# kpreid/all-is-cubes

Hardware: AMD Instinct MI355X
Metric: Mrays/s (higher is better)
Workload: dtype f64

## Files before the change

all_is_cubes_amd/csrc/aic_abi.cpp:

```cpp

#include <hip/hip_runtime.h>

#include <chrono>
#include <cmath>
#include <condition_variable>
#include <mutex>
#include <thread>
#include <cstdio>
#include <cstdlib>
#include <cstring>
#include <initializer_list>
#include <string>
#include <utility>
#include <vector>

#include "../../include/aic_hip.h"
#include "aic_bloom.h"
#include "aic_ctx.h"
#include "aic_device.h"
#include "aic_encode.h"
#include "aic_launch.h"

using namespace aic;

static_assert(sizeof(aic_pixel_aux) == sizeof(DevAux), "aux record layout");

static_assert(sizeof(aic_block_desc) == 48, "aic_block_desc is 48 bytes");

namespace {

constexpr uint64_t kMaxPoolElems = 0x7ffffff0ull;
constexpr uint64_t kMaxLightTexels = 0x3ffffff0ull;

}

namespace aic {

aic_options default_options() {
    aic_options o;
    std::memset(&o, 0, sizeof(o));
    o.fog = 1;
    o.transparency = 1;
    o.threshold = 0.5f;
    o.lighting = 3;
    o.maximum_intensity = INFINITY;
    o.bloom_intensity = 0.125f;
    o.view_distance = 200.0;
    return o;
}

void dump_record(aic_ctx *c, uint32_t tag, uint32_t layer, std::initializer_list<DumpPart> parts) {
    if (!c || !c->dump) return;
    uint64_t total = 0;
    for (const DumpPart &d : parts) total += d.p ? d.n : 0;
    std::fwrite(&tag, 4, 1, c->dump);
    std::fwrite(&layer, 4, 1, c->dump);
    std::fwrite(&total, 8, 1, c->dump);
    for (const DumpPart &d : parts)
        if (d.p && d.n) std::fwrite(d.p, 1, d.n, c->dump);
    std::fflush(c->dump);
}

thread_local std::string *tl_err_sink = nullptr;
int fail(aic_ctx *c, int code, const char *what, hipError_t e) {
    if (c) {
        std::string &dst = tl_err_sink ? *tl_err_sink : c->err;
        dst = what;
        if (e != hipSuccess) {
            dst += ": ";
            dst += hipGetErrorString(e);
        }
    }
    return code;
}

int hip_fail(aic_ctx *c, const char *what, hipError_t e) {
    return fail(c, e == hipErrorOutOfMemory ? AIC_ERR_OOM : AIC_ERR_DEVICE, what, e);
}

int take_light_spare(aic_ctx *c, Layer &l, int layer, size_t n, int *index) {
    auto in_use = [&](const DevBuf<uint32_t> &b) {
        for (uint32_t i = 0; i < AIC_MAX_IN_FLIGHT; i++)
            if (c->slots[i].busy && b.p && c->slots[i].light_used[layer] == (const void *)b.p) return true;
        return false;
    };
    int pick = -1;
    for (int k = 0; k < Layer::kLightSpares && pick < 0; k++)
        if (l.light_spare[k].p && l.light_spare[k].cap >= n && !in_use(l.light_spare[k])) pick = k;
    for (int k = 0; k < Layer::kLightSpares && pick < 0; k++)
        if (!l.light_spare[k].p || (l.light_spare[k].cap < n && !in_use(l.light_spare[k]))) pick = k;
    if (pick < 0) {
        pick = 0;
        for (uint32_t i = 0; i < AIC_MAX_IN_FLIGHT; i++)
            if (c->slots[i].busy && c->slots[i].light_used[layer] == (const void *)l.light_spare[0].p) {
                const hipError_t e = hipStreamSynchronize(c->slots[i].stream);
                if (e != hipSuccess) return fail(c, AIC_ERR_DEVICE, "waiting for a frame that reads a spare light volume", e);
            }
    }
    const hipError_t e = l.light_spare[pick].ensure(n);
    if (e != hipSuccess) return fail(c, e == hipErrorOutOfMemory ? AIC_ERR_OOM : AIC_ERR_DEVICE, "alloc light (spare volume)", e);
    *index = pick;
    return AIC_OK;
}

int quiesce(aic_ctx *c) {
    { const int rc = light_job_finish(c); if (rc != AIC_OK) return rc; }
    for (uint32_t i = 0; i < AIC_MAX_IN_FLIGHT; i++)
        if (c->slots[i].busy) HIP_TRY(c, hipStreamSynchronize(c->slots[i].stream));
    return AIC_OK;
}

}

namespace {

bool valid_resolution(int r) { return r >= 1 && r <= 128 && (r & (r - 1)) == 0; }

inline uint32_t block_class(const DevBlock &b) { return (b.kind & 255u) ? 2u : ((b.kind & 0x80000000u) ? 0u : 1u); }
inline void set_class(std::vector<uint32_t> &cls, uint32_t index, uint32_t c2) {
    if (cls.size() <= index / 16u) cls.resize(index / 16u + 1u, 0u);
    cls[index / 16u] = (cls[index / 16u] & ~(3u << ((index & 15u) * 2u))) | (c2 << ((index & 15u) * 2u));
}

inline bool invisible(const float *e) { return e[3] == 0.f && e[4] == 0.f && e[5] == 0.f && e[6] == 0.f; }
inline bool selectable_float_ok(float v) {
    uint32_t bits;
    std::memcpy(&bits, &v, sizeof(bits));
    return bits == 0u || bits == 0x3f800000u;
}

int convert_block(aic_ctx *c, const aic_block_desc &d, const uint16_t *voxels, const float *palette, uint32_t vox_off,
                  uint32_t pal_off, DevBlock *out, std::vector<uint16_t> *vox_out, std::vector<DevPaletteEntry> *pal_out) {
    std::memset(out, 0, sizeof(*out));
    if (!valid_resolution(d.resolution)) return fail(c, AIC_ERR_INVALID, "block resolution must be a power of two in 1..128");
    const bool one = (d.flags & AIC_BLOCK_ONE) != 0;
    const bool voxel_flag = (d.flags & AIC_BLOCK_VOXEL_SELECTABLE) != 0;
    size_t nvox = one ? 1 : (size_t)d.vsize[0] * (size_t)d.vsize[1] * (size_t)d.vsize[2];
    for (int a = 0; a < 3 && !one; a++) {
        if (d.vsize[a] < 0 || d.vlo[a] < 0 || d.vlo[a] + d.vsize[a] > d.resolution)
            return fail(c, AIC_ERR_INVALID, "block voxel bounds exceed GridAab::for_block(resolution)");
    }
    if (d.pal_len == 0 && nvox > 0) return fail(c, AIC_ERR_INVALID, "block has voxels but an empty palette");
    if (!palette && (one || d.pal_len > 0)) return fail(c, AIC_ERR_INVALID, "block has a palette length but no palette");
    if (!voxels && !one && nvox > 0) return fail(c, AIC_ERR_INVALID, "block has a voxel volume but no voxels");
    for (uint32_t i = 0; i < (one ? 1u : d.pal_len) && palette; i++) {
        const float *e = palette + 8 * (size_t)i;
        for (int k = 0; k < 7; k++)
            if (!(e[k] >= 0.f)) return fail(c, AIC_ERR_INVALID, "palette entry has a negative or NaN component");
        if (!(e[3] <= 1.f)) return fail(c, AIC_ERR_INVALID, "palette entry has alpha above 1");
        if (voxel_flag && !selectable_float_ok(e[7])) return fail(c, AIC_ERR_INVALID, "palette entry of an AIC_BLOCK_VOXEL_SELECTABLE block: the eighth float is neither 1.0f nor 0.0f");
    }
    const bool block_selectable = !(d.flags & (AIC_BLOCK_UNSELECTABLE | AIC_BLOCK_AIR));
    auto voxel_selectable = [&](const float *e) { return voxel_flag ? e[7] == 1.f : !invisible(e); };
    if (one || d.resolution == 1) {
        const float *e = nullptr;
        static const float air[8] = {0, 0, 0, 0, 0, 0, 0, 0};
        if (one) e = palette;
        else {
            bool inb = nvox > 0 && d.vlo[0] <= 0 && d.vlo[1] <= 0 && d.vlo[2] <= 0 && d.vlo[0] + d.vsize[0] > 0 &&
                       d.vlo[1] + d.vsize[1] > 0 && d.vlo[2] + d.vsize[2] > 0;
            if (inb) {
                size_t i = ((size_t)(0 - d.vlo[0]) * d.vsize[1] + (size_t)(0 - d.vlo[1])) * d.vsize[2] + (size_t)(0 - d.vlo[2]);
                uint16_t idx = voxels[i];
                if (idx >= d.pal_len) return fail(c, AIC_ERR_INVALID, "voxel index exceeds palette");
                e = palette + 8 * (size_t)idx;
            } else e = air;
        }
        out->kind = invisible(e) ? 0x80000000u : 0u;
        for (int k = 0; k < 4; k++) out->color[k] = e[k] + 0.0f;
        for (int k = 0; k < 3; k++) out->emission[k] = e[4 + k] + 0.0f;
        out->pad[0] = block_selectable && voxel_selectable(e) ? kBlockSelectable : 0u;
        return AIC_OK;
    }
    std::vector<uint32_t> remap(d.pal_len);
    uint32_t n_inv = 0;
    for (uint32_t i = 0; i < d.pal_len; i++)
        if (invisible(palette + 8 * (size_t)i)) n_inv++;
    uint32_t next_inv = 0, next_vis = n_inv;
    size_t pal_base = pal_out->size();
    pal_out->resize(pal_base + d.pal_len);
    for (uint32_t i = 0; i < d.pal_len; i++) {
        const float *e = palette + 8 * (size_t)i;
        uint32_t dst = invisible(e) ? next_inv++ : next_vis++;
        remap[i] = dst;
        DevPaletteEntry &pe = (*pal_out)[pal_base + dst];
        for (int k = 0; k < 4; k++) pe.color[k] = e[k] + 0.0f;
        for (int k = 0; k < 3; k++) pe.emission[k] = e[4 + k] + 0.0f;
        pe.pad = voxel_selectable(e) ? 1.f : 0.f;
    }
    size_t vox_base = vox_out->size();
    vox_out->resize(vox_base + nvox);
    for (size_t i = 0; i < nvox; i++) {
        uint16_t idx = voxels[i];
        if (idx >= d.pal_len) return fail(c, AIC_ERR_INVALID, "voxel index exceeds palette");
        (*vox_out)[vox_base + i] = (uint16_t)remap[idx];
    }
    out->kind = (uint32_t)d.resolution;
    out->vlo_packed = (uint32_t)d.vlo[0] | ((uint32_t)d.vlo[1] << 8) | ((uint32_t)d.vlo[2] << 16);
    out->vsize_packed = (uint32_t)d.vsize[0] | ((uint32_t)d.vsize[1] << 8) | ((uint32_t)d.vsize[2] << 16);
    out->vox_off = vox_off;
    out->pal_off = pal_off;
    out->n_invisible = n_inv;
    out->pad[0] = block_selectable ? kBlockSelectable : 0u;
    return AIC_OK;
}

}

extern "C" {

int aic_abi_version(void) { return AIC_ABI_VERSION; }

aic_ctx *aic_create(int device_id, int *status) {
    int st_dummy;
    if (!status) status = &st_dummy;
    int n = 0;
    hipError_t e = hipGetDeviceCount(&n);
    if (e != hipSuccess || n <= 0) {
        *status = AIC_ERR_NO_DEVICE;
        return nullptr;
    }
    if (device_id < 0) {
        if (hipGetDevice(&device_id) != hipSuccess) device_id = 0;
    }
    if (device_id >= n) {
        *status = AIC_ERR_INVALID;
        return nullptr;
    }
    if (hipSetDevice(device_id) != hipSuccess) {
        *status = AIC_ERR_DEVICE;
        return nullptr;
    }
    aic_ctx *c = new aic_ctx();
    c->device = device_id;
    hipDeviceProp_t prop;
    if (hipGetDeviceProperties(&prop, device_id) == hipSuccess) c->n_cus = prop.multiProcessorCount > 0 ? (uint32_t)prop.multiProcessorCount : 256u;
    if (hipGetDeviceProperties(&prop, device_id) == hipSuccess) std::snprintf(c->devname, sizeof(c->devname), "%s (%s)", prop.name, prop.gcnArchName);
    {
        auto env_int = [](const char *name, int dflt) { const char *e = std::getenv(name); return e ? std::atoi(e) : dflt; };
        c->sw.tile = env_int("AIC_TILE", 0);
        c->sw.macro = env_int("AIC_MACRO", 0);
        c->sw.feedback = env_int("AIC_TILE_FEEDBACK", 1) != 0;
        c->sw.wait_whole_stream = env_int("AIC_WAIT_WHOLE_STREAM", 0) != 0;
        c->sw.lines_clear_keys = env_int("AIC_LINES_CLEAR_KEYS", 0) != 0;
        c->sw.tiles_per_wave = (uint32_t)std::max(0, env_int("AIC_TILES_PER_WAVE", 0));
        if (const char *p = std::getenv("AIC_WAVE_PROF")) c->sw.wave_prof = p;
    }
    if (const char *path = std::getenv("AIC_DUMP")) {
        static int n_dumps = 0;
        std::string pth = path;
        if (n_dumps > 0) pth += "." + std::to_string(n_dumps);
        n_dumps++;
        c->dump = std::fopen(pth.c_str(), "wb");
        if (c->dump) std::fwrite("AICDUMP1", 1, 8, c->dump);
    }
    bool ok = hipStreamCreateWithFlags(&c->stream, hipStreamNonBlocking) == hipSuccess;
    for (uint32_t i = 0; ok && i < 8u && i < AIC_MAX_IN_FLIGHT; i++) {
        aic_ctx::FrameSlot &fs = c->slots[i];
        if (i == 0) fs.stream = c->stream;
        else ok = hipStreamCreateWithFlags(&fs.stream, hipStreamNonBlocking) == hipSuccess;
        ok = ok && hipEventCreate(&fs.ev0) == hipSuccess && hipEventCreate(&fs.ev1) == hipSuccess && hipEventCreate(&fs.ev2) == hipSuccess && fs.sub[0].counters.ensure(1) == hipSuccess;
    }
    ok = ok && hipStreamCreateWithFlags(&c->upload_stream, hipStreamNonBlocking) == hipSuccess;
    float lut[256];
    lut[0] = 0.f;
    for (int v = 1; v < 256; v++) {
        float arg = ((float)v - 144.0f) / 10.0f;
        lut[v] = (float)std::exp2((double)arg);
    }
    ok = ok && c->lut.ensure(256) == hipSuccess && hipMemcpy(c->lut.p, lut, sizeof(lut), hipMemcpyHostToDevice) == hipSuccess;
    {
        auto enc = [](float cc) -> int {
            float v = cc <= 0.0031308f ? cc * (323.f / 25.f) : (211.f * std::pow(cc, 5.f / 12.f) - 11.f) / 200.f;
            float r = std::round(v * 255.f);
            if (!(r > 0.f)) return 0;
            return r >= 255.f ? 255 : (int)r;
        };
        float thr[256];
        thr[0] = 0.f;
        for (int k = 1; k < 256; k++) {
            uint32_t lo_b = 0u, hi_b = 0x40000000u;
            while (hi_b - lo_b > 1u) {
                const uint32_t mid = lo_b + (hi_b - lo_b) / 2u;
                float f;
                std::memcpy(&f, &mid, 4);
                if (enc(f) >= k) hi_b = mid; else lo_b = mid;
            }
            for (int back = 0; back < 8 && hi_b > 1u; back++) {
                uint32_t probe = hi_b - 1u;
                float f;
                std::memcpy(&f, &probe, 4);
                bool lower_found = false;
                for (uint32_t d = 0; d < 8u && probe > d; d++) {
                    const uint32_t q = probe - d;
                    std::memcpy(&f, &q, 4);
                    if (enc(f) >= k) { hi_b = q; lower_found = true; }
                }
                if (!lower_found) break;
            }
            std::memcpy(&thr[k], &hi_b, 4);
        }
        ok = ok && c->srgb_thr.ensure(256) == hipSuccess && hipMemcpy(c->srgb_thr.p, thr, sizeof(thr), hipMemcpyHostToDevice) == hipSuccess;
        uint32_t buckets[kSrgbBucketWords];
        ok = ok && srgb8_bucket_build(thr, buckets) && c->srgb_buckets.ensure(kSrgbBucketWords) == hipSuccess &&
             hipMemcpy(c->srgb_buckets.p, buckets, sizeof(buckets), hipMemcpyHostToDevice) == hipSuccess;
    }
    if (!ok) {
        *status = AIC_ERR_DEVICE;
        aic_destroy(c);
        return nullptr;
    }
    for (auto &l : c->layers) l.opt = default_options();
    *status = AIC_OK;
    return c;
}

void aic_destroy(aic_ctx *c) {
    if (!c) return;
    (void)hipSetDevice(c->device);
    (void)light_job_finish(c);
    if (c->ljob.worker.joinable()) {
        { std::lock_guard<std::mutex> lk(c->ljob.mu); c->ljob.quit = true; }
        c->ljob.cv.notify_all();
        c->ljob.worker.join();
    }
    if (c->stream) (void)hipStreamSynchronize(c->stream);
    for (uint32_t i = 0; i < AIC_MAX_IN_FLIGHT; i++) {
        aic_ctx::FrameSlot &fs = c->slots[i];
        if (fs.stream) (void)hipStreamSynchronize(fs.stream);
        for (auto &sb : fs.sub) sb.release();
        fs.ray_cold.release(); fs.edges.release();
        if (fs.ev0) (void)hipEventDestroy(fs.ev0);
        if (fs.ev1) (void)hipEventDestroy(fs.ev1);
        if (fs.ev2) (void)hipEventDestroy(fs.ev2);
        fs.tile_static.release(); fs.queue_static.release();
        if (i > 0 && fs.stream) (void)hipStreamDestroy(fs.stream);
    }
    for (auto &l : c->layers) l.release();
    c->lut.release(); c->srgb_thr.release(); c->srgb_buckets.release(); c->out.release(); c->aux.release(); c->staging.release(); c->ortho_views.release(); c->reproject_scratch.release(); c->pick_scratch.release(); c->stale_scratch.release(); c->stale_cubes_scratch.release(); c->present_scratch.release(); c->lines_scratch.release();
    c->text_atlas.release(); c->text_codes.release(); c->export_counts.release(); c->exposure_scratch.release(); c->cursor_scratch.release();
    if (c->dump) std::fclose(c->dump);
    if (c->upload_stream) (void)hipStreamDestroy(c->upload_stream);
    if (c->stream) (void)hipStreamDestroy(c->stream);
    delete c;
}

const char *aic_last_error(const aic_ctx *c) { return c ? c->err.c_str() : "no context"; }

int aic_device_name(const aic_ctx *c, char *buf, uint32_t buf_len) {
    if (!c || !buf || !buf_len) return AIC_ERR_INVALID;
    std::snprintf(buf, buf_len, "%s", c->devname);
    return AIC_OK;
}

int aic_upload_space(aic_ctx *c, int layer, const aic_space_desc *s) {
    if (!c || !s || !valid_layer(layer)) return fail(c, AIC_ERR_INVALID, "aic_upload_space: bad argument");
    HIP_TRY(c, hipSetDevice(c->device));
    { int qrc = quiesce(c); if (qrc != AIC_OK) return qrc; }
    for (int a = 0; a < 3; a++)
        if (s->size[a] < 0 || (int64_t)s->lo[a] + s->size[a] > 2147483647LL) return fail(c, AIC_ERR_INVALID, "space bounds out of range");
    Layer &l = c->layers[layer];
    const size_t n = (size_t)s->size[0] * (size_t)s->size[1] * (size_t)s->size[2];
    if (n && (!s->block_index || !s->light)) return fail(c, AIC_ERR_INVALID, "space has cubes but no block_index/light");
    if (s->n_blocks > 65536) return fail(c, AIC_ERR_INVALID, "more than 65536 blocks");
    if (n + s->n_voxels > kMaxPoolElems) return fail(c, AIC_ERR_INVALID, "space too large (cube grid + voxel pool must stay within 4 GiB)");
    if (n > kMaxLightTexels) return fail(c, AIC_ERR_INVALID, "space too large (the light volume, 4 bytes per cube, must stay within 4 GiB)");
    if (s->n_blocks && !s->blocks) return fail(c, AIC_ERR_INVALID, "blocks is null");
    for (int o = 0; o < 8; o++)
        for (int k = 0; k < 3; k++)
            if (!(s->sky[o][k] >= 0.f)) return fail(c, AIC_ERR_INVALID, "sky colour has a negative or NaN component");

    std::vector<DevBlock> blocks(s->n_blocks);
    std::vector<uint32_t> vox_cap(s->n_blocks, 0u), pal_cap(s->n_blocks, 0u), vox_base(s->n_blocks, 0u), pal_base(s->n_blocks, 0u);
    std::vector<uint16_t> vox;
    std::vector<DevPaletteEntry> pal;
    vox.reserve((size_t)s->n_voxels);
    pal.reserve((size_t)s->n_palette);
    int32_t air_index = -1;
    for (uint32_t i = 0; i < s->n_blocks; i++) {
        const aic_block_desc &d = s->blocks[i];
        const bool one = (d.flags & AIC_BLOCK_ONE) != 0;
        size_t nvox = one ? 1 : (size_t)(d.vsize[0] > 0 ? d.vsize[0] : 0) * (size_t)(d.vsize[1] > 0 ? d.vsize[1] : 0) * (size_t)(d.vsize[2] > 0 ? d.vsize[2] : 0);
        if ((uint64_t)d.vox_off + nvox > s->n_voxels || (uint64_t)d.pal_off + d.pal_len > s->n_palette)
            return fail(c, AIC_ERR_INVALID, "block voxel/palette range exceeds the pools");
        if (n + vox.size() + nvox > kMaxPoolElems || pal.size() + d.pal_len > 0xfffffff0ull) return fail(c, AIC_ERR_INVALID, "pool too large");
        const size_t vb = vox.size(), pb = pal.size();
        int rc = convert_block(c, d, s->voxels ? s->voxels + d.vox_off : nullptr, s->palette ? s->palette + 8 * (size_t)d.pal_off : nullptr,
                               (uint32_t)(n + vox.size()), (uint32_t)pal.size(), &blocks[i], &vox, &pal);
        if (rc != AIC_OK) return rc;
        vox_cap[i] = (uint32_t)(vox.size() - vb);
        pal_cap[i] = (uint32_t)(pal.size() - pb);
        vox_base[i] = (uint32_t)(n + vb);
        pal_base[i] = (uint32_t)pb;
        if ((d.flags & AIC_BLOCK_AIR) && air_index < 0) air_index = (int32_t)i;
    }
    for (size_t i = 0; i < n; i++)
        if (s->block_index[i] >= s->n_blocks) return fail(c, AIC_ERR_INVALID, "cube block index out of range");

    hipError_t e;
    std::vector<uint32_t> cls;
    for (uint32_t i = 0; i < s->n_blocks; i++) set_class(cls, i, block_class(blocks[i]));
    if (cls.empty()) cls.push_back(0u);
    if ((e = l.pool.ensure(n + vox.size())) != hipSuccess) return hip_fail(c, "alloc pool", e);
    if ((e = l.cls.ensure(cls.size())) != hipSuccess) return hip_fail(c, "alloc classes", e);
    if ((e = l.light.ensure(n)) != hipSuccess) return hip_fail(c, "alloc light", e);
    if ((e = l.blocks.ensure(blocks.size())) != hipSuccess) return hip_fail(c, "alloc blocks", e);
    if ((e = l.palette.ensure(pal.size())) != hipSuccess) return hip_fail(c, "alloc palette", e);
    if (n) {
        HIP_TRY(c, hipMemcpyAsync(l.pool.p, s->block_index, n * sizeof(uint16_t), hipMemcpyHostToDevice, c->stream));
        HIP_TRY(c, hipMemcpyAsync(l.light.p, s->light, n * 4, hipMemcpyHostToDevice, c->stream));
    }
    if (!blocks.empty()) HIP_TRY(c, hipMemcpyAsync(l.blocks.p, blocks.data(), blocks.size() * sizeof(DevBlock), hipMemcpyHostToDevice, c->stream));
    if (!vox.empty()) HIP_TRY(c, hipMemcpyAsync(l.pool.p + n, vox.data(), vox.size() * sizeof(uint16_t), hipMemcpyHostToDevice, c->stream));
    HIP_TRY(c, hipMemcpyAsync(l.cls.p, cls.data(), cls.size() * sizeof(uint32_t), hipMemcpyHostToDevice, c->stream));
    const bool cls_in_code = s->n_blocks <= kCubeIndexMask + 1u;
    if (cls_in_code) {
        launch_tag_cubes(l.pool.p, n, l.cls.p, 0, 1, c->stream);
        launch_open_cubes(l.pool.p, s->size, c->stream);
    }
    if (!pal.empty()) HIP_TRY(c, hipMemcpyAsync(l.palette.p, pal.data(), pal.size() * sizeof(DevPaletteEntry), hipMemcpyHostToDevice, c->stream));
    HIP_TRY(c, hipStreamSynchronize(c->stream));

    for (int a = 0; a < 3; a++) { l.lo[a] = s->lo[a]; l.size[a] = s->size[a]; }
    l.host_blocks.swap(blocks);
    l.host_cls.swap(cls);
    l.vox_cap.swap(vox_cap);
    l.pal_cap.swap(pal_cap);
    l.vox_base.swap(vox_base);
    l.pal_base.swap(pal_base);
    l.garbage_vox = l.garbage_pal = 0;
    l.air_index = air_index;
    l.sky_kind = s->sky_kind;
    for (int o = 0; o < 8; o++)
        for (int k = 0; k < 3; k++) l.sky[o][k] = s->sky[o][k] + 0.0f;
    for (int f = 0; f < 7; f++)
        l.block_sky[f] = (uint32_t)s->block_sky[f][0] | ((uint32_t)s->block_sky[f][1] << 8) | ((uint32_t)s->block_sky[f][2] << 16) |
                         ((uint32_t)s->block_sky[f][3] << 24);
    l.cls_in_code = cls_in_code;
    l.present = true;
    l.version++;
    l.upload_serial++;
    if (c->dump) {
        struct { int32_t lo[3], size[3]; uint32_t n_blocks; int32_t sky_kind; uint64_t n_voxels, n_palette; float sky[8][3]; uint8_t block_sky[7][4]; } h;
        std::memset(&h, 0, sizeof(h));
        for (int a = 0; a < 3; a++) { h.lo[a] = s->lo[a]; h.size[a] = s->size[a]; }
        h.n_blocks = s->n_blocks; h.sky_kind = s->sky_kind; h.n_voxels = s->n_voxels; h.n_palette = s->n_palette;
        std::memcpy(h.sky, s->sky, sizeof(h.sky));
        std::memcpy(h.block_sky, s->block_sky, sizeof(h.block_sky));
        dump_record(c, DUMP_UPLOAD, (uint32_t)layer,
                    {{&h, sizeof(h)}, {s->block_index, n * 2}, {s->light, n * 4}, {s->blocks, (size_t)s->n_blocks * sizeof(aic_block_desc)},
                     {s->voxels, (size_t)s->n_voxels * 2}, {s->palette, (size_t)s->n_palette * 32}});
    }
    return AIC_OK;
}

int aic_clear_space(aic_ctx *c, int layer) {
    if (!c || !valid_layer(layer)) return fail(c, AIC_ERR_INVALID, "aic_clear_space: bad argument");
    { int qrc = quiesce(c); if (qrc != AIC_OK) return qrc; }
    c->layers[layer].present = false;
    dump_record(c, DUMP_CLEAR, (uint32_t)layer, {});
    return AIC_OK;
}

int aic_update_cubes(aic_ctx *c, int layer, uint32_t n, const int32_t *xyz, const uint16_t *block_index, const uint8_t *light) {
    if (!c || !valid_layer(layer) || (n && !xyz)) return fail(c, AIC_ERR_INVALID, "aic_update_cubes: bad argument");
    Layer &l = c->layers[layer];
    if (!l.present) return fail(c, AIC_ERR_INVALID, "aic_update_cubes: no space uploaded for this layer");
    if (!n) return AIC_OK;
    HIP_TRY(c, hipSetDevice(c->device));
    { int qrc = quiesce(c); if (qrc != AIC_OK) return qrc; }
    if (block_index)
        for (uint32_t i = 0; i < n; i++)
            if (block_index[i] >= l.host_blocks.size()) return fail(c, AIC_ERR_INVALID, "cube block index out of range");
    const size_t b_xyz = (size_t)n * 12, b_bi = block_index ? (((size_t)n * 2 + 15) & ~(size_t)15) : 0, b_lt = light ? (size_t)n * 4 : 0;
    hipError_t e = c->staging.ensure(b_xyz + b_bi + b_lt + 64);
    if (e != hipSuccess) return hip_fail(c, "alloc staging", e);
    unsigned char *base = c->staging.p;
    HIP_TRY(c, hipMemcpyAsync(base, xyz, b_xyz, hipMemcpyHostToDevice, c->stream));
    if (block_index) HIP_TRY(c, hipMemcpyAsync(base + b_xyz, block_index, (size_t)n * 2, hipMemcpyHostToDevice, c->stream));
    if (light) HIP_TRY(c, hipMemcpyAsync(base + b_xyz + b_bi, light, b_lt, hipMemcpyHostToDevice, c->stream));
    l.version++;
    light_state_cubes_updated(l.lstate, l.version - 1, l.version, n, xyz, block_index, light);
    launch_scatter_cubes(l.pool.p, l.light.p, (const int32_t *)base, block_index ? (const uint16_t *)(base + b_xyz) : nullptr,
                         light ? (const uint32_t *)(base + b_xyz + b_bi) : nullptr, n, l.lo, l.size, l.cls_in_code ? l.cls.p : nullptr, c->stream);
    if (block_index && l.cls_in_code) launch_open_changed_cubes(l.pool.p, (const int32_t *)base, n, l.lo, l.size, c->stream);
    HIP_TRY(c, hipGetLastError());
    HIP_TRY(c, hipStreamSynchronize(c->stream));
    {
        const uint32_t h[4] = {n, block_index ? 1u : 0u, light ? 1u : 0u, 0u};
        dump_record(c, DUMP_CUBES, (uint32_t)layer, {{h, sizeof(h)}, {xyz, (size_t)n * 12}, {block_index, (size_t)n * 2}, {light, (size_t)n * 4}});
    }
    return AIC_OK;
}

int aic_probe_cube_grid(aic_ctx *c, int layer, uint16_t *out_grid, uint32_t *out_cls, uint32_t *out_tagged) {
    if (!c || !valid_layer(layer) || !out_grid) return fail(c, AIC_ERR_INVALID, "aic_probe_cube_grid: bad argument");
    Layer &l = c->layers[layer];
    if (!l.present) return fail(c, AIC_ERR_INVALID, "aic_probe_cube_grid: no space uploaded for this layer");
    HIP_TRY(c, hipSetDevice(c->device));
    { int qrc = quiesce(c); if (qrc != AIC_OK) return qrc; }
    const size_t n = l.n_cubes(), n_words = (l.host_blocks.size() + 15u) / 16u;
    if (n) HIP_TRY(c, hipMemcpy(out_grid, l.pool.p, n * sizeof(uint16_t), hipMemcpyDeviceToHost));
    if (out_cls && n_words) HIP_TRY(c, hipMemcpy(out_cls, l.cls.p, n_words * sizeof(uint32_t), hipMemcpyDeviceToHost));
    if (out_tagged) *out_tagged = l.cls_in_code ? 1u : 0u;
    return AIC_OK;
}

int aic_update_light_volume(aic_ctx *c, int layer, const uint8_t *light) {
    if (!c || !valid_layer(layer) || !light) return fail(c, AIC_ERR_INVALID, "aic_update_light_volume: bad argument");
    Layer &l = c->layers[layer];
    if (!l.present) return fail(c, AIC_ERR_INVALID, "aic_update_light_volume: no space uploaded for this layer");
    HIP_TRY(c, hipSetDevice(c->device));
    { const int rc = light_job_finish(c); if (rc != AIC_OK) return rc; }
    const size_t n = l.n_cubes();
    int spare = 0;
    { const int rc = take_light_spare(c, l, layer, n, &spare); if (rc != AIC_OK) return rc; }
    if (n) HIP_TRY(c, hipMemcpyAsync(l.light_spare[spare].p, light, n * 4, hipMemcpyHostToDevice, c->upload_stream));
    HIP_TRY(c, hipStreamSynchronize(c->upload_stream));
    std::swap(l.light, l.light_spare[spare]);
    l.version++;
    {
        const uint64_t h = n;
        dump_record(c, DUMP_LIGHT, (uint32_t)layer, {{&h, sizeof(h)}, {light, n * 4}});
    }
    return AIC_OK;
}

namespace {

int compact_pools(aic_ctx *c, Layer &l) {
    l.version++;
    const size_t n = l.n_cubes();
    uint64_t need_vox = n, need_pal = 0;
    for (size_t i = 0; i < l.host_blocks.size(); i++) { need_vox += l.vox_cap[i]; need_pal += l.pal_cap[i]; }
    DevBuf<uint16_t> np;
    DevBuf<DevPaletteEntry> npal;
    hipError_t e;
    if ((e = np.ensure((size_t)need_vox)) != hipSuccess) return hip_fail(c, "compact pool", e);
    if ((e = npal.ensure((size_t)(need_pal ? need_pal : 1))) != hipSuccess) { np.release(); return hip_fail(c, "compact palette", e); }
    std::vector<DevBlock> blocks = l.host_blocks;
    std::vector<uint32_t> vbase = l.vox_base, pbase = l.pal_base;
    uint64_t vo = n, po = 0;
    e = n ? hipMemcpyAsync(np.p, l.pool.p, n * sizeof(uint16_t), hipMemcpyDeviceToDevice, c->stream) : hipSuccess;
    for (size_t i = 0; e == hipSuccess && i < blocks.size(); i++) {
        DevBlock &b = blocks[i];
        if (l.vox_cap[i]) {
            e = hipMemcpyAsync(np.p + vo, l.pool.p + l.vox_base[i], (size_t)l.vox_cap[i] * sizeof(uint16_t), hipMemcpyDeviceToDevice, c->stream);
            if ((b.kind & 255u) != 0u) b.vox_off = (uint32_t)vo;
            vbase[i] = (uint32_t)vo;
            vo += l.vox_cap[i];
        }
        if (e == hipSuccess && l.pal_cap[i]) {
            e = hipMemcpyAsync(npal.p + po, l.palette.p + l.pal_base[i], (size_t)l.pal_cap[i] * sizeof(DevPaletteEntry), hipMemcpyDeviceToDevice, c->stream);
            if ((b.kind & 255u) != 0u) b.pal_off = (uint32_t)po;
            pbase[i] = (uint32_t)po;
            po += l.pal_cap[i];
        }
    }
    if (e == hipSuccess && !blocks.empty())
        e = hipMemcpyAsync(l.blocks.p, blocks.data(), blocks.size() * sizeof(DevBlock), hipMemcpyHostToDevice, c->stream);
    if (e == hipSuccess) e = hipStreamSynchronize(c->stream);
    if (e != hipSuccess) {
        if (!l.host_blocks.empty()) (void)hipMemcpy(l.blocks.p, l.host_blocks.data(), l.host_blocks.size() * sizeof(DevBlock), hipMemcpyHostToDevice);
        np.release();
        npal.release();
        return hip_fail(c, "compact pools", e);
    }
    l.pool.release();
    l.palette.release();
    l.pool = np;
    l.palette = npal;
    l.pool.n = (size_t)vo;
    l.palette.n = (size_t)po;
    l.host_blocks.swap(blocks);
    l.vox_base.swap(vbase);
    l.pal_base.swap(pbase);
    l.garbage_vox = l.garbage_pal = 0;
    return AIC_OK;
}

int replace_one(aic_ctx *c, int layer, Layer &l, uint32_t index, const aic_block_desc *desc, const uint16_t *voxels, const float *palette) {
    l.version++;
    if (!desc) return fail(c, AIC_ERR_INVALID, "aic_replace_block: null descriptor");
    if (index > l.host_blocks.size() || index >= 65536) return fail(c, AIC_ERR_INVALID, "aic_replace_block: index out of range");
    const bool exists = index < l.host_blocks.size();
    std::vector<uint16_t> vox;
    std::vector<DevPaletteEntry> pal;
    DevBlock db;
    int rc = convert_block(c, *desc, voxels, palette, 0u, 0u, &db, &vox, &pal);
    if (rc != AIC_OK) return rc;
    const bool fits = exists && vox.size() <= l.vox_cap[index] && pal.size() <= l.pal_cap[index];
    uint32_t vox_off, pal_off;
    hipError_t e;
    if (fits) {
        vox_off = l.vox_base[index];
        pal_off = l.pal_base[index];
    } else {
        vox_off = (uint32_t)l.pool.n;
        pal_off = (uint32_t)l.palette.n;
        if ((uint64_t)vox_off + vox.size() > kMaxPoolElems || (uint64_t)pal_off + pal.size() > 0xfffffff0ull)
            return fail(c, AIC_ERR_INVALID, "voxel pool too large");
        if (!vox.empty() && (e = l.pool.ensure(vox_off + vox.size(), true, c->stream)) != hipSuccess) return hip_fail(c, "grow pool", e);
        if (!pal.empty() && (e = l.palette.ensure(pal_off + pal.size(), true, c->stream)) != hipSuccess) return hip_fail(c, "grow palette", e);
        if (exists) { l.garbage_vox += l.vox_cap[index]; l.garbage_pal += l.pal_cap[index]; }
    }
    if (!vox.empty()) {
        db.vox_off = vox_off;
        HIP_TRY(c, hipMemcpy(l.pool.p + vox_off, vox.data(), vox.size() * sizeof(uint16_t), hipMemcpyHostToDevice));
    }
    if (!pal.empty()) {
        db.pal_off = pal_off;
        HIP_TRY(c, hipMemcpy(l.palette.p + pal_off, pal.data(), pal.size() * sizeof(DevPaletteEntry), hipMemcpyHostToDevice));
    }
    bool class_changed = false;
    if (!exists) {
        l.host_blocks.push_back(db);
        l.vox_cap.push_back((uint32_t)vox.size());
        l.pal_cap.push_back((uint32_t)pal.size());
        l.vox_base.push_back(vox_off);
        l.pal_base.push_back(pal_off);
        if ((e = l.blocks.ensure(l.host_blocks.size(), true, c->stream)) != hipSuccess) return hip_fail(c, "grow blocks", e);
    } else {
        class_changed = block_class(l.host_blocks[index]) != block_class(db);
        l.host_blocks[index] = db;
        if (!fits) {
            l.vox_cap[index] = (uint32_t)vox.size(); l.pal_cap[index] = (uint32_t)pal.size();
            l.vox_base[index] = vox_off; l.pal_base[index] = pal_off;
        }
    }
    HIP_TRY(c, hipMemcpy(l.blocks.p + index, &db, sizeof(db), hipMemcpyHostToDevice));
    set_class(l.host_cls, index, block_class(db));
    if ((e = l.cls.ensure(l.host_cls.size(), true, c->stream)) != hipSuccess) return hip_fail(c, "grow classes", e);
    HIP_TRY(c, hipMemcpy(l.cls.p + index / 16u, &l.host_cls[index / 16u], sizeof(uint32_t), hipMemcpyHostToDevice));
    if (l.cls_in_code) {
        if (l.host_blocks.size() > kCubeIndexMask + 1u) {
            launch_tag_cubes(l.pool.p, l.n_cubes(), l.cls.p, 1, 0, c->stream);
            l.cls_in_code = false;
        } else if (class_changed) {
            launch_tag_cubes(l.pool.p, l.n_cubes(), l.cls.p, 1, 1, c->stream);
            launch_open_cubes(l.pool.p, l.size, c->stream);
        }
        HIP_TRY(c, hipGetLastError());
    }
    if (desc->flags & AIC_BLOCK_AIR) {
        if (l.air_index < 0) l.air_index = (int32_t)index;
    } else if (l.air_index == (int32_t)index) {
        l.air_index = -1;
    }
    {
        const bool one = (desc->flags & AIC_BLOCK_ONE) != 0;
        const uint64_t nvox = one ? 0 : (uint64_t)(desc->vsize[0] > 0 ? desc->vsize[0] : 0) * (uint64_t)(desc->vsize[1] > 0 ? desc->vsize[1] : 0) * (uint64_t)(desc->vsize[2] > 0 ? desc->vsize[2] : 0);
        const uint64_t h[2] = {index, nvox};
        dump_record(c, DUMP_BLOCK, (uint32_t)layer, {{h, sizeof(h)}, {desc, sizeof(*desc)}, {voxels, (size_t)nvox * 2}, {palette, (size_t)desc->pal_len * 32}});
    }
    return AIC_OK;
}

}

int aic_replace_blocks(aic_ctx *c, int layer, uint32_t n, const uint32_t *indices, const aic_block_desc *descs, const uint16_t *const *voxels,
                       const float *const *palettes) {
    if (!c || !valid_layer(layer) || (n && (!indices || !descs || !voxels || !palettes))) return fail(c, AIC_ERR_INVALID, "aic_replace_blocks: bad argument");
    Layer &l = c->layers[layer];
    if (!l.present) return fail(c, AIC_ERR_INVALID, "aic_replace_block: no space uploaded for this layer");
    HIP_TRY(c, hipSetDevice(c->device));
    { int qrc = quiesce(c); if (qrc != AIC_OK) return qrc; }
    int rc = AIC_OK;
    for (uint32_t k = 0; k < n && rc == AIC_OK; k++) rc = replace_one(c, layer, l, indices[k], &descs[k], voxels[k], palettes[k]);
    HIP_TRY(c, hipStreamSynchronize(c->stream));
    if (rc != AIC_OK) return rc;
    const bool big_vox = l.garbage_vox * 4 > l.pool.n && l.garbage_vox > (1u << 17);
    const bool big_pal = l.garbage_pal * 4 > l.palette.n && l.garbage_pal > (1u << 13);
    if (big_vox || big_pal) return compact_pools(c, l);
    return AIC_OK;
}

int aic_compact(aic_ctx *c, int layer) {
    if (!c || !valid_layer(layer)) return fail(c, AIC_ERR_INVALID, "aic_compact: bad argument");
    Layer &l = c->layers[layer];
    if (!l.present) return AIC_OK;
    HIP_TRY(c, hipSetDevice(c->device));
    { int qrc = quiesce(c); if (qrc != AIC_OK) return qrc; }
    return compact_pools(c, l);
}

int aic_replace_block(aic_ctx *c, int layer, uint32_t index, const aic_block_desc *desc, const uint16_t *voxels, const float *palette) {
    if (!desc) return fail(c, AIC_ERR_INVALID, "aic_replace_block: bad argument");
    return aic_replace_blocks(c, layer, 1u, &index, desc, &voxels, &palette);
}

int aic_set_options(aic_ctx *c, int layer, const aic_options *o) {
    if (!c || !valid_layer(layer) || !o) return fail(c, AIC_ERR_INVALID, "aic_set_options: bad argument");
    if (o->fog < 0 || o->fog > 3 || o->transparency < 0 || o->transparency > 2 || o->lighting < 0 || o->lighting > 5 ||
        o->antialiasing < 0 || o->antialiasing > 2 || o->tone_mapping < 0 || o->tone_mapping > 1 || !(o->view_distance > 0.0))
        return fail(c, AIC_ERR_INVALID, "aic_set_options: enum or view_distance out of range");
    c->layers[layer].opt = *o;
    c->layers[layer].opt_set = true;
    dump_record(c, DUMP_OPTIONS, (uint32_t)layer, {{o, sizeof(*o)}});
    return AIC_OK;
}

int aic_set_depth_transform(aic_ctx *c, const double zw[4]) {
    if (!c || !zw) return fail(c, AIC_ERR_INVALID, "aic_set_depth_transform: bad argument");
    for (int i = 0; i < 4; i++)
        if (!std::isfinite(zw[i])) return fail(c, AIC_ERR_INVALID, "aic_set_depth_transform: a component is not finite");
    HIP_TRY(c, hipSetDevice(c->device));
    { const int rc = quiesce(c); if (rc != AIC_OK) return rc; }
    std::memcpy(c->depth_zw, zw, sizeof(c->depth_zw));
    return AIC_OK;
}

uint32_t aic_partition_rows(uint32_t height, const aic_partition *p) {
    if (!p || p->n_parts <= 1 || p->strip_rows == 0) return height;
    if (p->part >= p->n_parts) return 0;
    uint32_t rows = 0;
    const uint32_t n_strips = (height + p->strip_rows - 1) / p->strip_rows;
    for (uint32_t s = p->part; s < n_strips; s += p->n_parts) {
        uint32_t r0 = s * p->strip_rows;
        uint32_t r1 = r0 + p->strip_rows;
        if (r1 > height) r1 = height;
        rows += r1 - r0;
    }
    return rows;
}

int aic_assemble_strips_on(aic_ctx *c, const void *gathered_device, void *out_device, uint32_t width, uint32_t height,
                           uint32_t strip_rows, uint32_t n_parts, void *hip_stream) {
    if (!c || !gathered_device || !out_device || !strip_rows || !n_parts) return fail(c, AIC_ERR_INVALID, "aic_assemble_strips: bad argument");
    HIP_TRY(c, hipSetDevice(c->device));
    uint32_t max_rows = 0;
    for (uint32_t p = 0; p < n_parts; p++) {
        aic_partition pp = {strip_rows, n_parts, p, 0};
        uint32_t r = aic_partition_rows(height, &pp);
        if (r > max_rows) max_rows = r;
    }
    launch_assemble_strips((const uint32_t *)gathered_device, (uint32_t *)out_device, width, height, strip_rows, n_parts, max_rows, hip_stream ? (hipStream_t)hip_stream : c->stream);
    HIP_TRY(c, hipGetLastError());
    return AIC_OK;
}

int aic_assemble_strips_async(aic_ctx *c, const void *gathered_device, void *out_device, uint32_t width, uint32_t height,
                              uint32_t strip_rows, uint32_t n_parts) {
    return aic_assemble_strips_on(c, gathered_device, out_device, width, height, strip_rows, n_parts, nullptr);
}

int aic_assemble_strips(aic_ctx *c, const void *gathered_device, void *out_device, uint32_t width, uint32_t height,
                        uint32_t strip_rows, uint32_t n_parts) {
    const int rc = aic_assemble_strips_async(c, gathered_device, out_device, width, height, strip_rows, n_parts);
    if (rc != AIC_OK) return rc;
    HIP_TRY(c, hipStreamSynchronize(c->stream));
    return AIC_OK;
}

int aic_read_aux(aic_ctx *c, aic_pixel_aux *out, uint64_t n_records) {
    if (!c || !out) return fail(c, AIC_ERR_INVALID, "aic_read_aux: bad argument");
    if (n_records > c->aux_records) return fail(c, AIC_ERR_INVALID, "aic_read_aux: more records requested than the last frame produced");
    HIP_TRY(c, hipSetDevice(c->device));
    HIP_TRY(c, hipMemcpy(out, c->aux.p, n_records * sizeof(aic_pixel_aux), hipMemcpyDeviceToHost));
    return AIC_OK;
}

int aic_synchronize(aic_ctx *c) {
    if (!c) return AIC_ERR_INVALID;
    HIP_TRY(c, hipSetDevice(c->device));
    HIP_TRY(c, hipStreamSynchronize(c->stream));
    for (uint32_t i = 1; i < AIC_MAX_IN_FLIGHT; i++)
        if (c->slots[i].stream) HIP_TRY(c, hipStreamSynchronize(c->slots[i].stream));
    return AIC_OK;
}

void *aic_stream(aic_ctx *c) { return c ? (void *)c->stream : nullptr; }

int aic_wait_event(aic_ctx *c, void *hip_event) {
    if (!c || !hip_event) return fail(c, AIC_ERR_INVALID, "aic_wait_event: bad argument");
    HIP_TRY(c, hipSetDevice(c->device));
    HIP_TRY(c, hipStreamWaitEvent(c->stream, (hipEvent_t)hip_event, 0));
    for (uint32_t i = 1; i < AIC_MAX_IN_FLIGHT; i++)
        if (c->slots[i].stream) HIP_TRY(c, hipStreamWaitEvent(c->slots[i].stream, (hipEvent_t)hip_event, 0));
    return AIC_OK;
}

int aic_stream_wait_frame(aic_ctx *c, uint32_t slot, void *hip_stream) {
    if (!c || slot >= AIC_MAX_IN_FLIGHT) return fail(c, AIC_ERR_INVALID, "aic_stream_wait_frame: bad argument");
    HIP_TRY(c, hipSetDevice(c->device));
    aic_ctx::FrameSlot &fs = c->slots[slot];
    if (!fs.busy || !fs.npix) return AIC_OK;
    HIP_TRY(c, hipStreamWaitEvent((hipStream_t)hip_stream, fs.ev1, 0));
    return AIC_OK;
}

int aic_probe_raycast(aic_ctx *c, const double origin[3], const double direction[3], int use_bounds, const int32_t lo[3],
                      const int32_t hi[3], int include_exit, uint32_t max_steps, aic_rc_step *out, uint32_t *n_out, int *ended) {
    if (!c || !origin || !direction || !out || !n_out || !ended) return fail(c, AIC_ERR_INVALID, "aic_probe_raycast: bad argument");
    HIP_TRY(c, hipSetDevice(c->device));
    const size_t bytes = 6 * sizeof(double) + 8 * sizeof(int) + (size_t)max_steps * 8 * sizeof(double) + 64;
    hipError_t e = c->staging.ensure(bytes);
    if (e != hipSuccess) return hip_fail(c, "alloc staging", e);
    unsigned char *base = c->staging.p;
    double od[6] = {origin[0], origin[1], origin[2], direction[0], direction[1], direction[2]};
    int lohi[8] = {0, 0, 0, 0, 0, 0, 0, 0};
    if (use_bounds && lo && hi) {
        for (int a = 0; a < 3; a++) { lohi[a] = lo[a]; lohi[3 + a] = hi[a]; }
    }
    double *d_od = (double *)base;
    int *d_lohi = (int *)(base + 48);
    uint32_t *d_n = (uint32_t *)(base + 48 + 24);
    int *d_end = (int *)(base + 48 + 28);
    double *d_rec = (double *)(base + 48 + 32);
    HIP_TRY(c, hipMemcpyAsync(d_od, od, sizeof(od), hipMemcpyHostToDevice, c->stream));
    HIP_TRY(c, hipMemcpyAsync(d_lohi, lohi, 24, hipMemcpyHostToDevice, c->stream));
    launch_probe_raycast(d_od, use_bounds, d_lohi, include_exit, max_steps, d_rec, d_n, d_end, c->stream);
    HIP_TRY(c, hipGetLastError());
    std::vector<double> rec((size_t)max_steps * 8);
    uint32_t n = 0;
    int en = 0;
    HIP_TRY(c, hipMemcpyAsync(&n, d_n, 4, hipMemcpyDeviceToHost, c->stream));
    HIP_TRY(c, hipMemcpyAsync(&en, d_end, 4, hipMemcpyDeviceToHost, c->stream));
    if (max_steps) HIP_TRY(c, hipMemcpyAsync(rec.data(), d_rec, rec.size() * sizeof(double), hipMemcpyDeviceToHost, c->stream));
    HIP_TRY(c, hipStreamSynchronize(c->stream));
    for (uint32_t i = 0; i < n && i < max_steps; i++) {
        const double *r = rec.data() + 8 * (size_t)i;
        out[i].cube[0] = (int32_t)r[0]; out[i].cube[1] = (int32_t)r[1]; out[i].cube[2] = (int32_t)r[2];
        out[i].face = (int32_t)r[3];
        out[i].t_distance = r[4];
        out[i].intersection_point[0] = r[5]; out[i].intersection_point[1] = r[6]; out[i].intersection_point[2] = r[7];
    }
    *n_out = n;
    *ended = en;
    return AIC_OK;
}

int aic_probe_powf(aic_ctx *c, const float *x, const float *y, uint32_t n, float *out) {
    if (!c || (n && (!x || !y || !out))) return fail(c, AIC_ERR_INVALID, "aic_probe_powf: bad argument");
    if (!n) return AIC_OK;
    HIP_TRY(c, hipSetDevice(c->device));
    hipError_t e = c->staging.ensure((size_t)n * 12);
    if (e != hipSuccess) return hip_fail(c, "alloc staging", e);
    float *dx = (float *)c->staging.p, *dy = dx + n, *dout = dy + n;
    HIP_TRY(c, hipMemcpyAsync(dx, x, (size_t)n * 4, hipMemcpyHostToDevice, c->stream));
    HIP_TRY(c, hipMemcpyAsync(dy, y, (size_t)n * 4, hipMemcpyHostToDevice, c->stream));
    launch_probe_powf(dx, dy, dout, n, c->stream);
    HIP_TRY(c, hipGetLastError());
    HIP_TRY(c, hipMemcpyAsync(out, dout, (size_t)n * 4, hipMemcpyDeviceToHost, c->stream));
    HIP_TRY(c, hipStreamSynchronize(c->stream));
    return AIC_OK;
}

int aic_probe_expf(aic_ctx *c, const float *x, uint32_t n, float *out) {
    if (!c || (n && (!x || !out))) return fail(c, AIC_ERR_INVALID, "aic_probe_expf: bad argument");
    if (!n) return AIC_OK;
    for (uint32_t i = 0; i < n; i++)
        if (!(std::fabs(x[i]) < 88.0f)) return fail(c, AIC_ERR_INVALID, "aic_probe_expf: x outside (-88, 88)");
    HIP_TRY(c, hipSetDevice(c->device));
    hipError_t e = c->staging.ensure((size_t)n * 8);
    if (e != hipSuccess) return hip_fail(c, "alloc staging", e);
    float *dx = (float *)c->staging.p, *dout = dx + n;
    HIP_TRY(c, hipMemcpyAsync(dx, x, (size_t)n * 4, hipMemcpyHostToDevice, c->stream));
    launch_probe_expf(dx, dout, n, c->stream);
    HIP_TRY(c, hipGetLastError());
    HIP_TRY(c, hipMemcpyAsync(out, dout, (size_t)n * 4, hipMemcpyDeviceToHost, c->stream));
    HIP_TRY(c, hipStreamSynchronize(c->stream));
    return AIC_OK;
}

int aic_probe_bloom(aic_ctx *c, uint32_t width, uint32_t height, const float *colorbuf, float exposure, const aic_options *options, uint8_t *out_rgba8,
                    uint16_t *out_mip0, uint32_t mip0_size[2]) {
    if (!c || !colorbuf || !options || !out_rgba8 || !width || !height) return fail(c, AIC_ERR_INVALID, "aic_probe_bloom: bad argument");
    if (width > 65535u || height > 65535u) return fail(c, AIC_ERR_INVALID, "aic_probe_bloom: frame dimensions above 65535 are not supported");
    if (!(exposure >= 0.f) || !(options->bloom_intensity >= 0.f)) return fail(c, AIC_ERR_INVALID, "aic_probe_bloom: exposure or bloom_intensity is negative or NaN");
    HIP_TRY(c, hipSetDevice(c->device));
    if (c->slots[0].busy) return fail(c, AIC_ERR_INVALID, "aic_probe_bloom: a submitted frame still occupies slot 0 (aic_render_wait it first)");
    const BloomGeom geom = bloom_geometry(width, height);
    const size_t npix = (size_t)width * height;
    aic_ctx::SubSlot &sb = c->slots[0].sub[0];
    hipError_t e;
    if ((e = sb.bloom_cb.ensure(npix)) != hipSuccess || (e = sb.bloom_mips.ensure(geom.texels)) != hipSuccess || (e = c->out.ensure(npix)) != hipSuccess)
        return hip_fail(c, "alloc bloom scratch", e);
    HIP_TRY(c, hipMemcpyAsync(sb.bloom_cb.p, colorbuf, npix * 16, hipMemcpyHostToDevice, c->stream));
    BloomParams bp;
    bp.colorbuf = sb.bloom_cb.p;
    bp.mips = sb.bloom_mips.p;
    bp.out = c->out.p;
    bp.exposure = exposure + 0.0f;
    bp.intensity = options->bloom_intensity;
    bp.tone_mapping = options->tone_mapping;
    bp.maximum_intensity = options->maximum_intensity;
    bp.srgb_thr = c->srgb_thr.p;
    launch_bloom(geom, bp, c->stream);
    HIP_TRY(c, hipGetLastError());
    HIP_TRY(c, hipMemcpyAsync(out_rgba8, c->out.p, npix * 4, hipMemcpyDeviceToHost, c->stream));
    if (out_mip0) HIP_TRY(c, hipMemcpyAsync(out_mip0, sb.bloom_mips.p, (size_t)geom.mw[0] * geom.mh[0] * 8, hipMemcpyDeviceToHost, c->stream));
    HIP_TRY(c, hipStreamSynchronize(c->stream));
    if (mip0_size) { mip0_size[0] = geom.mw[0]; mip0_size[1] = geom.mh[0]; }
    return AIC_OK;
}

int aic_probe_light_lut(aic_ctx *c, float out[256]) {
    if (!c || !out) return AIC_ERR_INVALID;
    HIP_TRY(c, hipSetDevice(c->device));
    HIP_TRY(c, hipMemcpy(out, c->lut.p, 256 * sizeof(float), hipMemcpyDeviceToHost));
    return AIC_OK;
}

}
```

all_is_cubes_amd/csrc/aic_colour.h:

```cpp
#pragma once

#include <hip/hip_runtime.h>
#include <stdint.h>

#include "aic_encode.h"

namespace aic {


AIC_DEV float zo_clamped(float v) {
    if (v > 0.f && v <= 1.f) return v;
    if (v <= 0.f) return 0.f;
    return 1.f;
}

__device__ const double kPowLog2Tab[16][2] = {
    {0x1.661ec79f8f3bep+0, -0x1.efec65b963019p-2}, {0x1.571ed4aaf883dp+0, -0x1.b0b6832d4fca4p-2},
    {0x1.49539f0f010bp+0, -0x1.7418b0a1fb77bp-2},  {0x1.3c995b0b80385p+0, -0x1.39de91a6dcf7bp-2},
    {0x1.30d190c8864a5p+0, -0x1.01d9bf3f2b631p-2}, {0x1.25e227b0b8eap+0, -0x1.97c1d1b3b7afp-3},
    {0x1.1bb4a4a1a343fp+0, -0x1.2f9e393af3c9fp-3}, {0x1.12358f08ae5bap+0, -0x1.960cbbf788d5cp-4},
    {0x1.0953f419900a7p+0, -0x1.a6f9db6475fcep-5}, {0x1p+0, 0x0p+0},
    {0x1.e608cfd9a47acp-1, 0x1.338ca9f24f53dp-4},  {0x1.ca4b31f026aap-1, 0x1.476a9543891bap-3},
    {0x1.b2036576afce6p-1, 0x1.e840b4ac4e4d2p-3},  {0x1.9c2d163a1aa2dp-1, 0x1.40645f0c6651cp-2},
    {0x1.886e6037841edp-1, 0x1.88e9c2c1b9ff8p-2},  {0x1.767dcf5534862p-1, 0x1.ce0a44eb17bccp-2},
};
__device__ const unsigned long long kPowExp2Tab[32] = {
    0x3ff0000000000000ull, 0x3fefd9b0d3158574ull, 0x3fefb5586cf9890full, 0x3fef9301d0125b51ull,
    0x3fef72b83c7d517bull, 0x3fef54873168b9aaull, 0x3fef387a6e756238ull, 0x3fef1e9df51fdee1ull,
    0x3fef06fe0a31b715ull, 0x3feef1a7373aa9cbull, 0x3feedea64c123422ull, 0x3feece086061892dull,
    0x3feebfdad5362a27ull, 0x3feeb42b569d4f82ull, 0x3feeab07dd485429ull, 0x3feea47eb03a5585ull,
    0x3feea09e667f3bcdull, 0x3fee9f75e8ec5f74ull, 0x3feea11473eb0187ull, 0x3feea589994cce13ull,
    0x3feeace5422aa0dbull, 0x3feeb737b0cdc5e5ull, 0x3feec49182a3f090ull, 0x3feed503b23e255dull,
    0x3feee89f995ad3adull, 0x3feeff76f2fb5e47ull, 0x3fef199bdd85529cull, 0x3fef3720dcef9069ull,
    0x3fef5818dcfba487ull, 0x3fef7c97337b9b5full, 0x3fefa4afa2a490daull, 0x3fefd0765b6e4540ull,
};
AIC_DEV void pow_tables_to_lds(double *s_pow, uint32_t tid, uint32_t nthreads) {
    for (uint32_t i = tid; i < 64u; i += nthreads)
        s_pow[i] = i < 32u ? kPowLog2Tab[i >> 1][i & 1u] : __longlong_as_double((long long)kPowExp2Tab[i - 32u]);
}
AIC_DEV bool powf_table_domain(float x, float y) {
    const uint32_t ix = __float_as_uint(x), iy = __float_as_uint(y);
    return ix >= 0x00800000u && ix < 0x3f800000u && iy > 0u && iy < 0x7f800000u;
}
AIC_DEV double KC(double v) { asm volatile("" : "+s"(v)); return v; }
AIC_DEV float powf_table(float x, float y, const double *s_pow) {
    const uint32_t ix = __float_as_uint(x);
    const uint32_t tmp = ix - 0x3f330000u;
    const uint32_t i = (tmp >> 19) & 15u;
    const uint32_t top = tmp & 0xff800000u;
    const uint32_t iz = ix - top;
    const int k = (int)top >> 23;
    const double invc = s_pow[2u * i], logc = s_pow[2u * i + 1u];
    const double z = (double)__uint_as_float(iz);
    const double r = fma(z, invc, -1.0);
    const double y0 = logc + (double)k;
    const double r2 = r * r;
    double yy = fma(KC(0x1.27616c9496e0bp-2), r, KC(-0x1.71969a075c67ap-2));
    const double pp = fma(KC(0x1.ec70a6ca7baddp-2), r, KC(-0x1.7154748bef6c8p-1));
    const double r4 = r2 * r2;
    double q = fma(KC(0x1.71547652ab82bp+0), r, y0);
    q = fma(pp, r2, q);
    yy = fma(yy, r4, q);
    const double ylogx = (double)y * yy;
    if (ylogx <= -150.0) return 0.0f;
    double kd = ylogx + KC(0x1.8p+47);
    const unsigned long long ki = (unsigned long long)__double_as_longlong(kd);
    kd -= KC(0x1.8p+47);
    const double rr = ylogx - kd;
    unsigned long long t = (unsigned long long)__double_as_longlong(s_pow[32u + (uint32_t)(ki & 31u)]);
    t += ki << 47;
    const double sc = __longlong_as_double((long long)t);
    const double zz = fma(KC(0x1.c6af84b912394p-5), rr, KC(0x1.ebfce50fac4f3p-3));
    const double rr2 = rr * rr;
    double e = fma(KC(0x1.62e42ff0c52d6p-1), rr, 1.0);
    e = fma(zz, rr2, e);
    e = e * sc;
    return (float)e;
}
AIC_DEV float expf_table(float x, const double *s_pow) {
    const double z = KC(0x1.71547652b82fep+5) * (double)x;
    double kd = z + KC(0x1.8p+52);
    const unsigned long long ki = (unsigned long long)__double_as_longlong(kd);
    kd -= KC(0x1.8p+52);
    const double r = z - kd;
    unsigned long long t = (unsigned long long)__double_as_longlong(s_pow[32u + (uint32_t)(ki & 31u)]);
    t += ki << 47;
    const double sc = __longlong_as_double((long long)t);
    const double zz = fma(KC(0x1.c6af84b912394p-20), r, KC(0x1.ebfce50fac4f3p-13));
    const double r2 = r * r;
    double y = fma(KC(0x1.62e42ff0c52d6p-6), r, 1.0);
    y = fma(zz, r2, y);
    y = y * sc;
    return (float)y;
}

AIC_DEV void cb_add(ColorBuf &b, float s0, float s1, float s2, float st) {
    b.l0 += s0 * b.t;
    b.l1 += s1 * b.t;
    b.l2 += s2 * b.t;
    b.t *= st;
}
AIC_DEV bool cb_opaque(const ColorBuf &b) { return b.t < 1.0f / 256.0f; }

}
```

all_is_cubes_amd/csrc/aic_ctx.h:

```cpp
#pragma once

#include <hip/hip_runtime.h>

#include <chrono>
#include <condition_variable>
#include <cstdio>
#include <initializer_list>
#include <mutex>
#include <string>
#include <thread>
#include <vector>

#include "../../include/aic_hip.h"
#include "aic_device.h"

namespace aic {

template <typename T>
struct DevBuf {
    T *p = nullptr;
    size_t n = 0;
    size_t cap = 0;
    hipError_t ensure(size_t count, bool keep = false, hipStream_t stream = nullptr) {
        if (count <= cap) { n = count; return hipSuccess; }
        size_t new_cap = count + count / 4 + 16;
        T *np_ = nullptr;
        hipError_t e = hipMalloc((void **)&np_, new_cap * sizeof(T));
        if (e != hipSuccess) return e;
        if (keep && p && cap) {
            e = hipMemcpyAsync(np_, p, cap * sizeof(T), hipMemcpyDeviceToDevice, stream);
            if (e == hipSuccess) e = hipStreamSynchronize(stream);
            if (e != hipSuccess) {
                (void)hipFree(np_);
                return e;
            }
        }
        if (p) (void)hipFree(p);
        p = np_;
        cap = new_cap;
        n = count;
        return hipSuccess;
    }
    void release() {
        if (p) (void)hipFree(p);
        p = nullptr;
        n = cap = 0;
    }
};

struct LightState;
void light_state_free(LightState *s);
void light_state_cubes_updated(LightState *s, uint64_t version_before, uint64_t version_after, uint32_t n, const int32_t *xyz, const uint16_t *block_index,
                               const uint8_t *light);

struct Layer {
    bool present = false;
    int32_t lo[3] = {0, 0, 0}, size[3] = {0, 0, 0};
    DevBuf<uint16_t> pool;
    DevBuf<uint32_t> cls;
    std::vector<uint32_t> host_cls;
    DevBuf<uint32_t> light;
    static constexpr int kLightSpares = 7;
    DevBuf<uint32_t> light_spare[kLightSpares];
    DevBuf<DevBlock> blocks;
    DevBuf<DevPaletteEntry> palette;
    std::vector<DevBlock> host_blocks;
    std::vector<uint32_t> vox_cap, pal_cap, vox_base, pal_base;
    uint64_t garbage_vox = 0, garbage_pal = 0;
    int32_t air_index = -1;
    int32_t sky_kind = 0;
    float sky[8][3] = {};
    uint32_t block_sky[7] = {};
    aic_options opt;
    bool opt_set = false;
    bool cls_in_code = false;
    uint64_t version = 0;
    uint64_t upload_serial = 0;
    LightState *lstate = nullptr;
    DevBuf<uint32_t> visible_bits;
    uint64_t visible_version = ~0ull;
    size_t n_cubes() const { return (size_t)size[0] * (size_t)size[1] * (size_t)size[2]; }
    void release() {
        pool.release(); cls.release(); light.release(); blocks.release(); palette.release(); visible_bits.release();
        visible_version = ~0ull;
        for (auto &sp : light_spare) sp.release();
        host_blocks.clear(); host_cls.clear(); vox_cap.clear(); pal_cap.clear(); vox_base.clear(); pal_base.clear();
        garbage_vox = garbage_pal = 0;
        present = false;
        version++;
        light_state_free(lstate);
        lstate = nullptr;
    }
};

}

using namespace aic;

struct aic_ctx {
    int device = 0;
    hipStream_t stream = nullptr;
    hipStream_t upload_stream = nullptr;
    Layer layers[2];
    DevBuf<float> lut;
    DevBuf<float> srgb_thr;
    DevBuf<uint32_t> srgb_buckets;
    DevBuf<uint32_t> out;
    DevBuf<DevAux> aux;
    DevBuf<unsigned char> staging;
    DevBuf<DevOrthoView> ortho_views;
    DevBuf<unsigned char> reproject_scratch;
    uint32_t reproject_valid_w = 0, reproject_valid_h = 0;
    DevBuf<uint32_t> pick_scratch;
    DevBuf<uint2> present_scratch;
    DevBuf<unsigned char> lines_scratch;
    size_t lines_keys_clean = 0;
    DevBuf<uint32_t> text_atlas;
    uint32_t text_cell_w = 0, text_cell_h = 0, text_margin = 0;
    bool text_space_blank = false;
    DevBuf<unsigned char> text_codes;
    DevBuf<unsigned char> exposure_scratch;
    DevBuf<uint32_t> export_counts;
    uint64_t aux_records = 0;
    double depth_zw[4] = {1.0, 0.0, 0.0, 1.0};
    bool streaming_submit = false;
    struct SubSlot {
        DevBuf<DevCounters> counters;
        DevCounters *host_counters = nullptr;
        bool counters_clean = false;
        size_t cost_clean_n = 0;
        bool record_ready = false;
        uint32_t order_key[6] = {0, 0, 0, 0, 0, 0};
        DevBuf<float4> acc;
        DevBuf<double> split_depth;
        DevBuf<uint32_t> tile_cost, tile_order, queue_start;
        DevBuf<float4> bloom_cb;
        DevBuf<uint2> bloom_mips;
        uint32_t cost_sig[4] = {0, 0, 0, 0};
        double cost_cam[16] = {0};
        void release() {
            counters.release(); acc.release(); split_depth.release(); tile_cost.release(); tile_order.release(); queue_start.release(); bloom_cb.release(); bloom_mips.release();
            if (host_counters) (void)hipHostFree(host_counters);
            host_counters = nullptr;
            counters_clean = record_ready = false; cost_clean_n = 0;
        }
    };
    struct FrameSlot {
        hipStream_t stream = nullptr;
        hipEvent_t ev0 = nullptr, ev1 = nullptr;
        hipEvent_t ev2 = nullptr;
        SubSlot sub[kMaxSub];
        uint32_t n_sub = 1;
        bool static_ready = false;
        uint32_t static_key[6] = {0, 0, 0, 0, 0, 0};
        DevBuf<uint32_t> tile_static, queue_static;
        DevBuf<uint4> ray_cold;
        DevBuf<double> edges;
        uint32_t edges_w = 0, edges_h = 0;
        bool busy = false;
        bool diag = false;
        uint32_t variant = 0, tile_queues = 0;
        const void *light_used[2] = {nullptr, nullptr};
        uint32_t flaws = 0, local_rows = 0;
        size_t npix = 0;
        std::chrono::steady_clock::time_point t_begin;
    } slots[AIC_MAX_IN_FLIGHT];
    std::string err;
    std::FILE *dump = nullptr;
    char devname[256] = {0};
    uint32_t n_cus = 256;
    struct LightJob {
        std::thread worker;
        std::mutex mu;
        std::condition_variable cv;
        bool has_work = false, quit = false;
        bool running = false;
        bool pending = false;
        bool result_ready = false;
        int layer = 0, spare = -1;
        aic_light_params params;
        std::vector<int32_t> queue_cubes, queue_priorities;
        int rc = AIC_OK;
        aic_light_info info;
        std::string err;
    } ljob;
    struct Switches {
        int tile = 0, macro = 0;
        bool feedback = true;
        bool wait_whole_stream = false;
        uint32_t tiles_per_wave = 0;
        std::string wave_prof;
        bool lines_clear_keys = false;
    } sw;
    DevBuf<unsigned char> stale_scratch;
    DevBuf<unsigned char> cursor_scratch;
    DevBuf<unsigned char> stale_cubes_scratch;
};

namespace aic {

extern thread_local std::string *tl_err_sink;
int fail(aic_ctx *c, int code, const char *what, hipError_t e = hipSuccess);
int hip_fail(aic_ctx *c, const char *what, hipError_t e);
inline int reject(aic_ctx *c, const char *who, const char *why) { return fail(c, AIC_ERR_INVALID, (std::string(who) + ": " + why).c_str()); }
#define HIP_TRY(ctx, expr)                                    \
    do {                                                      \
        hipError_t e_ = (expr);                               \
        if (e_ != hipSuccess) return hip_fail(ctx, #expr, e_); \
    } while (0)

inline bool valid_layer(int l) { return l == AIC_LAYER_WORLD || l == AIC_LAYER_UI; }

aic_options default_options();
enum DumpTag : uint32_t { DUMP_UPLOAD = 1, DUMP_CLEAR = 2, DUMP_CUBES = 3, DUMP_LIGHT = 4, DUMP_BLOCK = 5, DUMP_OPTIONS = 6, DUMP_FRAME = 7 };
struct DumpPart { const void *p; size_t n; };
void dump_record(aic_ctx *c, uint32_t tag, uint32_t layer, std::initializer_list<DumpPart> parts);
int take_light_spare(aic_ctx *c, Layer &l, int layer, size_t n, int *index);
int quiesce(aic_ctx *c);
int light_job_finish(aic_ctx *c);
constexpr uint32_t kVisibleBitsWords = 2048;
int light_visible_bits(aic_ctx *c, Layer &l, hipStream_t stream, std::vector<uint32_t> *bits);

}
```

all_is_cubes_amd/csrc/aic_device.h:

```cpp
#pragma once

#include <hip/hip_runtime.h>
#include <stdint.h>

namespace aic {

struct DevBlock {
    float color[4];
    float emission[3];
    uint32_t kind;
    uint32_t vlo_packed;
    uint32_t vsize_packed;
    uint32_t vox_off;
    uint32_t pal_off;
    uint32_t n_invisible;
    uint32_t pad[3];
};
static constexpr uint32_t kBlockSelectable = 1u;
static_assert(sizeof(DevBlock) == 64, "DevBlock is one 64-byte line");

struct DevPaletteEntry {
    float color[4];
    float emission[3];
    float pad;
};
static_assert(sizeof(DevPaletteEntry) == 32, "palette entry is 32 B");

struct DevOptions {
    int32_t fog;
    int32_t transparency;
    float threshold;
    int32_t lighting;
    int32_t antialiasing;
    int32_t debug_pixel_cost;
    int32_t tone_mapping;
    float maximum_intensity;
    int32_t bounce_samples;
    int32_t pad_;
    double view_distance;
};

struct DevLayer {
    const uint16_t *pool;
    const uint32_t *cls;
    const uint32_t *light;
    const DevBlock *blocks;
    const DevPaletteEntry *palette;
    int32_t lo[3];
    int32_t size[3];
    uint32_t n_blocks;
    int32_t present;
    int32_t air_index;
    int32_t sky_kind;
    float sky[8][3];
    uint32_t block_sky[7];
    DevOptions opt;
    double inv[16];
    float exposure;
    uint32_t cls_in_code;
};

static constexpr uint32_t kCubeClassShift = 14u;
static constexpr uint32_t kCubeIndexMask = (1u << kCubeClassShift) - 1u;
static constexpr uint32_t kCubeTagOpen = 0u, kCubeTagInvisible = 1u, kCubeTagVisible = 2u, kCubeTagRecursive = 3u;
__host__ __device__ inline uint32_t cube_entry_class(uint32_t entry) {
    const uint32_t tag = entry >> kCubeClassShift;
    return tag > kCubeTagInvisible ? tag - 1u : 0u;
}

constexpr uint32_t kMaxTileQueues = 8;

struct DevCounters {
    unsigned long long cubes_traced;
    unsigned long long n_outer;
    unsigned long long n_inner;
    unsigned long long n_hits;
    unsigned long long n_light;
    unsigned long long bailed;
    unsigned long long prof[48];
    uint32_t tile_next;
    uint32_t waves_done;
    uint32_t tile_next_q[kMaxTileQueues][16];
#ifdef AIC_PROFILE
    uint32_t wave_prof[2048][4];
#endif
};

struct DevAux {
    int32_t hit;
    int32_t cube[3];
    int32_t voxel[3];
    int32_t resolution;
    int32_t face;
    int32_t block_index;
    uint32_t cubes_traced;
    uint32_t layer;
    double t_distance;
};

struct DevOrthoView {
    uint32_t x0, y0, w, h;
    double m[16];
    double dir[3];
};

struct DevSub {
    double inv[16];
    float backdrop[4];
    float exposure;
    int32_t has_backdrop;
    uint32_t *out;
    float4 *acc_buf;
    DevCounters *counters;
    unsigned long long *host_counters;
    const uint32_t *tile_order;
    uint32_t *tile_cost;
    const uint32_t *queue_start;
};
constexpr uint32_t kMaxSub = 8;

struct DevFrame {
    DevLayer layer;
    int32_t layer_transparency, layer_lighting;
    uint32_t width, height;
    int32_t antialias;
    float maximum_intensity;
    int32_t tone_mapping;
    uint32_t strip_rows, n_parts, part;
    uint32_t local_rows;
    uint32_t tiles_x, tiles_y;
    uint32_t tile;
    uint32_t macro;
    uint32_t macros_x, macros_y;
    uint32_t n_cus;
    uint32_t tiles_per_wave;
    int32_t pass;
    uint32_t hit_layer;
    int32_t use_init;
    int32_t pixel_centers;
    int32_t out_mode;
    const DevOrthoView *ortho;
    int32_t ortho_n;
    const double *patches;
    uint32_t n_patches;
    int32_t bare_trace;
    const double *rays;
    DevAux *aux;
    uint32_t n_queues;
    uint32_t n_sub;
    DevSub sub[kMaxSub];
    const float *light_lut;
    const uint32_t *srgb_buckets;
    const double *edge_x, *edge_y;
    uint4 *ray_cold;
    uint32_t ray_cold_groups;
    uint32_t ray_mode;
    uint32_t exchange;
    double depth_zw[4];
    double *split_depth[kMaxSub];
    float split_ui_exposure[kMaxSub];
    const uint32_t *pixels;
    uint32_t px_width, px_height;
    uint32_t px_in_place;
};

struct OrderJobs {
    const uint32_t *cost[kMaxSub];
    uint32_t *order[kMaxSub];
    uint32_t *queue_start[kMaxSub];
    uint32_t *clear_words[kMaxSub];
};

constexpr int kTile = 16;
constexpr int kClsWords = 4096;

}
```

all_is_cubes_amd/csrc/aic_frame.cpp:

```cpp

#include <hip/hip_runtime.h>

#include <algorithm>
#include <chrono>
#include <cmath>
#include <cstdio>
#include <cstring>
#include <utility>
#include <vector>

#include "../../include/aic_hip.h"
#include "aic_bloom.h"
#include "aic_ctx.h"
#include "aic_device.h"
#include "aic_launch.h"

using namespace aic;

namespace {

void fill_dev_layer(const Layer &l, const aic_camera &cam, DevLayer *d) {
    std::memset(d, 0, sizeof(*d));
    d->present = l.present ? 1 : 0;
    d->pool = l.pool.p;
    d->cls = l.cls.p;
    d->n_blocks = (uint32_t)l.host_blocks.size();
    d->light = l.light.p;
    d->blocks = l.blocks.p;
    d->palette = l.palette.p;
    for (int a = 0; a < 3; a++) { d->lo[a] = l.lo[a]; d->size[a] = l.size[a]; }
    d->air_index = l.air_index;
    d->sky_kind = l.sky_kind;
    std::memcpy(d->sky, l.sky, sizeof(d->sky));
    std::memcpy(d->block_sky, l.block_sky, sizeof(d->block_sky));
    const aic_options o = l.opt_set ? l.opt : default_options();
    d->opt.fog = o.fog;
    d->opt.transparency = o.transparency;
    d->opt.threshold = o.threshold;
    d->opt.lighting = o.lighting;
    d->opt.bounce_samples = o.bounce_samples;
    d->opt.antialiasing = o.antialiasing;
    d->opt.debug_pixel_cost = o.debug_pixel_cost;
    d->opt.tone_mapping = o.tone_mapping;
    d->opt.maximum_intensity = o.maximum_intensity;
    d->opt.view_distance = o.view_distance;
    std::memcpy(d->inv, cam.inverse_projection_view, sizeof(d->inv));
    d->exposure = cam.exposure + 0.0f;
    d->cls_in_code = l.cls_in_code ? 1u : 0u;
}

bool cameras_close(const double a[16], const double b[16]) {
    auto unproject = [](const double m[16], double x, double y, double z, double out[3]) {
        const double w = x * m[3] + y * m[7] + z * m[11] + m[15];
        for (int k = 0; k < 3; k++) out[k] = (x * m[k] + y * m[4 + k] + z * m[8 + k] + m[12 + k]) / w;
    };
    static const double pts[3][2] = {{0.0, 0.0}, {1.0, 1.0}, {-1.0, -1.0}};
    for (const auto &p : pts) {
        double na[3], fa[3], nb[3], fb[3];
        unproject(a, p[0], p[1], 0.0, na); unproject(a, p[0], p[1], 1.0, fa);
        unproject(b, p[0], p[1], 0.0, nb); unproject(b, p[0], p[1], 1.0, fb);
        double da[3], db[3], la = 0, lb = 0, dot = 0, move = 0;
        for (int k = 0; k < 3; k++) {
            da[k] = fa[k] - na[k]; db[k] = fb[k] - nb[k];
            la += da[k] * da[k]; lb += db[k] * db[k]; dot += da[k] * db[k];
            move += (na[k] - nb[k]) * (na[k] - nb[k]);
        }
        if (!(la > 0) || !(lb > 0)) return false;
        if (!(dot / std::sqrt(la * lb) >= 0.99985)) return false;
        if (!(move <= 0.0625)) return false;
    }
    return true;
}

struct RayBatch {
    const double *rays;
    uint32_t n;
    bool no_sky;
    uint32_t layer;
    DevAux *aux_target;
};
struct PixelList {
    const uint32_t *pixels;
    uint32_t n, width, height;
    bool in_place;
    DevAux *aux_target;
};
struct Traced {
    const double *patches = nullptr;
    uint32_t n_patches = 0;
    const DevOrthoView *ortho = nullptr;
    int32_t ortho_n = 0;
    const RayBatch *rb = nullptr;
    const PixelList *px = nullptr;
    int world_seat = AIC_LAYER_WORLD;
    bool whole_frame() const { return !patches && !rb && !px && !ortho_n; }
    DevAux *aux_target() const { return rb ? rb->aux_target : (px ? px->aux_target : nullptr); }
};

struct FramePlan {
    aic_partition part;
    uint32_t local_rows = 0;
    size_t npix = 0;
    bool split = false, bloom = false, diag = false, want_aux = false, ui = false;
    uint32_t flaws = 0;
    uint32_t n_tiles = 0, n_queues = 0, sb_shift = 0;
    uint32_t sig[4] = {0, 0, 0, 0}, order_key[6] = {0, 0, 0, 0, 0, 0};
    bool use_feedback = false, ordered = false;
    size_t ray_cold_bytes = 0;
    uint32_t ray_cold_groups = 0;
    DevLayer hl[2];
    DevFrame F;
};

aic_partition normalised_partition(const aic_frame_desc &f) {
    aic_partition part = f.partition;
    if (part.n_parts <= 1 || part.strip_rows == 0) {
        part.n_parts = 1;
        part.part = 0;
        part.strip_rows = f.height ? f.height : 1;
    }
    return part;
}

int validate_frames(aic_ctx *c, uint32_t k, const aic_frame_desc *frames, uint32_t *const *out_devices, uint32_t slot, const Traced &what, FramePlan &P) {
    const aic_frame_desc *f = &frames[0];
    P.part = normalised_partition(*f);
    if (P.part.part >= P.part.n_parts) return fail(c, AIC_ERR_INVALID, "aic_render: partition.part >= n_parts");
    if (f->flags & AIC_FRAME_BLOOM) {
        if (f->flags & (AIC_FRAME_OUT_LINEAR | AIC_FRAME_OUT_COLORBUF)) return fail(c, AIC_ERR_INVALID, "aic_render: AIC_FRAME_BLOOM is for RGBA8 output only");
        if (P.part.n_parts > 1u) return fail(c, AIC_ERR_UNSUPPORTED, "aic_render: AIC_FRAME_BLOOM needs the whole frame (partition.n_parts = 1)");
        if (!what.whole_frame()) return fail(c, AIC_ERR_UNSUPPORTED, "AIC_FRAME_BLOOM: not for patches, rays or orthographic views");
    }
    P.split = (f->flags & AIC_FRAME_OUT_SPLIT) != 0;
    if (P.split && (f->flags & (AIC_FRAME_OUT_LINEAR | AIC_FRAME_OUT_COLORBUF | AIC_FRAME_BLOOM)))
        return fail(c, AIC_ERR_INVALID, "aic_render: AIC_FRAME_OUT_SPLIT excludes AIC_FRAME_OUT_LINEAR, AIC_FRAME_OUT_COLORBUF and AIC_FRAME_BLOOM");
    P.local_rows = aic_partition_rows(f->height, &P.part);
    P.npix = (size_t)f->width * P.local_rows;
    for (uint32_t j = 0; j < k; j++) {
        if (P.npix && !out_devices[j]) return fail(c, AIC_ERR_INVALID, "aic_render: output buffer is null");
        if (P.split && ((uintptr_t)out_devices[j] & 7u)) return fail(c, AIC_ERR_INVALID, "aic_render: an AIC_FRAME_OUT_SPLIT buffer starts at an 8-byte boundary");
    }
    if (!what.patches && !what.rb && !what.px)
        for (uint32_t j = 0; j < k; j++) dump_record(c, DUMP_FRAME, slot, {{&frames[j], sizeof(frames[j])}});
    if (f->width > 65535u || P.local_rows > 65535u) return fail(c, AIC_ERR_INVALID, "aic_render: frame dimensions above 65535 are not supported");
    for (uint32_t j = 0; j < k; j++)
        if (!(frames[j].world.exposure >= 0.f) || !(frames[j].ui.exposure >= 0.f)) return fail(c, AIC_ERR_INVALID, "aic_render: exposure is negative or NaN");
    return AIC_OK;
}

uint32_t part_grid_tiles_per_wave(const aic_ctx *c, uint32_t slot, const DevFrame &F) {
    uint32_t busy_others = 0;
    for (uint32_t i = 0; i < AIC_MAX_IN_FLIGHT; i++) busy_others += (i != slot && c->slots[i].busy && c->slots[i].npix) ? 1u : 0u;
    const uint32_t resident_waves = (uint32_t)c->n_cus * 16u;
    const uint32_t tpw_full = (F.tiles_x * F.tiles_y + resident_waves - 1u) / resident_waves;
    if (tpw_full >= 4u && busy_others > 0u) {
        const uint32_t t = tpw_full * (busy_others < 4u ? busy_others : 4u);
        return t < 32u ? t : (tpw_full > 32u ? tpw_full : 32u);
    }
    return F.tiles_per_wave;
}

void plan_geometry(const aic_ctx *c, uint32_t k, const aic_frame_desc *f, uint32_t slot, const Traced &what, FramePlan &P) {
    DevFrame &F = P.F;
    DevLayer *hl = P.hl;
    std::memset(&F, 0, sizeof(F));
    const Layer &seated = c->layers[what.world_seat];
    fill_dev_layer(seated, f->world, &hl[0]);
    fill_dev_layer(c->layers[AIC_LAYER_UI], f->ui, &hl[1]);
    const aic_options &bloom_opt = seated.opt;
    P.bloom = (f->flags & AIC_FRAME_BLOOM) && bloom_opt.bloom_intensity > 0.0f;
    if (bloom_opt.bloom_intensity != 0.0f && !P.bloom) P.flaws |= AIC_FLAW_NO_BLOOM;
    F.width = f->width;
    F.height = f->height;
    F.n_sub = k;
    F.pixel_centers = (f->flags & AIC_FRAME_PIXEL_CENTERS) && !what.patches ? 1 : 0;
    F.out_mode = P.split ? 3 : ((f->flags & AIC_FRAME_OUT_LINEAR) ? 1 : ((f->flags & AIC_FRAME_OUT_COLORBUF) || P.bloom ? 2 : 0));
    std::memcpy(F.depth_zw, c->depth_zw, sizeof(F.depth_zw));
    F.patches = what.patches;
    F.n_patches = what.rb ? what.rb->n : (what.px ? what.px->n : what.n_patches);
    if (what.px) {
        F.pixels = what.px->pixels;
        F.px_width = what.px->width;
        F.px_height = what.px->height;
        F.px_in_place = what.px->in_place ? 1u : 0u;
    }
    F.ortho = what.ortho;
    F.ortho_n = what.ortho_n;
    F.rays = what.rb ? what.rb->rays : nullptr;
    F.bare_trace = (what.ortho_n || what.rb) ? 1 : 0;
    if (what.rb) hl[1].present = 0;
    if (what.ortho_n) {
        hl[1].present = 0;
        DevOptions &o = hl[0].opt;
        o.fog = 0; o.transparency = 1; o.lighting = 0; o.antialiasing = 0; o.debug_pixel_cost = 0; o.tone_mapping = 0;
        o.maximum_intensity = INFINITY; o.view_distance = 200.0;
        hl[0].exposure = 1.0f;
        P.flaws = 0;
    }
    P.ui = hl[1].present != 0;
    F.antialias = (hl[0].opt.antialiasing == 2 && !F.pixel_centers && !what.rb) ? 1 : 0;
    F.maximum_intensity = hl[0].opt.maximum_intensity;
    F.tone_mapping = hl[0].opt.tone_mapping;
    F.strip_rows = P.part.strip_rows;
    F.n_parts = P.part.n_parts;
    F.part = P.part.part;
    F.local_rows = P.local_rows;
    {
        const int forced = c->sw.tile;
        F.tile = (forced == 8 || forced == 16) ? (uint32_t)forced : 8u;
        F.tiles_x = (f->width + F.tile - 1) / F.tile;
        F.tiles_y = (P.local_rows + F.tile - 1) / F.tile;
        const int macro_env = c->sw.macro;
        F.macro = (macro_env == 1 || macro_env == 2 || macro_env == 4 || macro_env == 8 || macro_env == 16) ? (uint32_t)macro_env : 2u;
        F.macros_x = (F.tiles_x + F.macro - 1) / F.macro;
        F.macros_y = (F.tiles_y + F.macro - 1) / F.macro;
    }
    F.light_lut = c->lut.p;
    F.n_cus = c->n_cus;
    F.tiles_per_wave = c->sw.tiles_per_wave ? c->sw.tiles_per_wave : (c->streaming_submit ? 4u : 1u);
    if (!c->sw.tiles_per_wave && c->streaming_submit && k == 1u) F.tiles_per_wave = part_grid_tiles_per_wave(c, slot, F);
    F.srgb_buckets = c->srgb_buckets.p;
}

void plan_dispatch(const aic_ctx *c, uint32_t k, const aic_frame_desc *f, bool allow_aux, const Traced &what, FramePlan &P) {
    DevFrame &F = P.F;
    P.want_aux = allow_aux && (f->flags & AIC_FRAME_AUX) != 0;
    P.diag = P.want_aux || P.split || what.px || (f->flags & AIC_FRAME_COUNTERS) != 0;
    P.n_tiles = F.macros_x * F.macros_y;
    const int queues_env = (int)((f->tuning >> AIC_TUNE_QUEUES_SHIFT) & 15u);
    const int super_env = (int)((f->tuning >> AIC_TUNE_SUPER_SHIFT) & 31u) - 1;
    P.n_queues = queues_env > 0 ? (uint32_t)queues_env : (uint32_t)c->n_cus / 32u;
    if (P.n_queues > kMaxTileQueues) P.n_queues = kMaxTileQueues;
    if (P.n_queues < 2u || !what.whole_frame() || !P.n_tiles) P.n_queues = 0u;
    const uint32_t macro_log2 = F.macro >= 16 ? 4u : (F.macro >= 8 ? 3u : (F.macro >= 4 ? 2u : (F.macro >= 2 ? 1u : 0u)));
    const uint32_t tile_log2 = F.tile >= 16 ? 4u : 3u;
    uint32_t sb_px_log2 = 0;
    while ((2u << sb_px_log2) <= std::max(1u, P.local_rows / 8u)) sb_px_log2++;
    P.sb_shift = super_env >= 0 ? (uint32_t)std::min(super_env, 12) : (sb_px_log2 > macro_log2 + tile_log2 ? sb_px_log2 - macro_log2 - tile_log2 : 0u);
    P.use_feedback = c->sw.feedback && P.n_tiles && what.whole_frame() && !(f->flags & AIC_FRAME_NO_FEEDBACK);
    const uint32_t sig[4] = {f->width, P.local_rows, (P.part.n_parts << 16) | P.part.part, (P.part.strip_rows << 8) | (F.macro << 4) | (F.tile >> 3)};
    const uint32_t order_key[6] = {sig[0], sig[1], sig[2], sig[3], P.n_queues, P.sb_shift};
    std::memcpy(P.sig, sig, sizeof(sig));
    std::memcpy(P.order_key, order_key, sizeof(order_key));
    P.ordered = P.use_feedback || P.n_queues;
    F.n_queues = P.ordered ? P.n_queues : 0u;
    if (!P.diag) {
        P.ray_cold_bytes = trace_ray_cold_bytes(c->n_cus, &P.ray_cold_groups);
        if (P.ray_cold_bytes) {
            const uint32_t asked = (f->tuning >> AIC_TUNE_VARIANT_SHIFT) & 3u;
            const double resident_waves = (double)c->n_cus * 16.0 / (double)k;
            const double need = c->streaming_submit ? 1.9 : 5.0;
            F.exchange = asked == AIC_VARIANT_EXCHANGING ? 1u : (asked == AIC_VARIANT_PLAIN ? 0u : (((double)F.tiles_x * (double)F.tiles_y >= need * resident_waves) ? 1u : 0u));
        }
    }
}

bool record_predicts(const FramePlan &P, const aic_ctx::SubSlot &sb, const aic_frame_desc &frame) {
    return P.use_feedback && sb.record_ready && std::memcmp(P.order_key, sb.order_key, sizeof(P.order_key)) == 0 && sb.tile_order.n >= P.n_tiles &&
           cameras_close(frame.world.inverse_projection_view, sb.cost_cam);
}

int ensure_static_order(aic_ctx *c, aic_ctx::FrameSlot &fs, uint32_t k, const aic_frame_desc *frames, const FramePlan &P) {
    if (!P.ordered || !P.n_queues) return AIC_OK;
    bool any_static = false;
    for (uint32_t j = 0; j < k; j++) any_static = any_static || !record_predicts(P, fs.sub[j], frames[j]);
    if (!any_static || (fs.static_ready && std::memcmp(P.order_key, fs.static_key, sizeof(P.order_key)) == 0 && fs.tile_static.n >= P.n_tiles)) return AIC_OK;
    fs.static_ready = false;
    hipError_t e;
    if ((e = fs.tile_static.ensure(P.n_tiles)) != hipSuccess || (e = fs.queue_static.ensure(kMaxTileQueues + 1)) != hipSuccess) return hip_fail(c, "alloc tile queues", e);
    launch_order_tiles(nullptr, fs.tile_static.p, P.n_tiles, P.F.macros_x, P.sb_shift, P.n_queues, fs.queue_static.p, fs.stream);
    HIP_TRY(c, hipGetLastError());
    std::memcpy(fs.static_key, P.order_key, sizeof(P.order_key));
    fs.static_ready = true;
    return AIC_OK;
}

int bind_sub_frame(aic_ctx *c, aic_ctx::FrameSlot &fs, uint32_t j, const aic_frame_desc &frame, uint32_t *out_device, FramePlan &P) {
    aic_ctx::SubSlot &sb = fs.sub[j];
    DevFrame &F = P.F;
    DevSub &S = F.sub[j];
    const uint32_t n_tiles = P.n_tiles;
    hipError_t e;
    std::memcpy(S.backdrop, frame.backdrop, sizeof(S.backdrop));
    S.has_backdrop = !(frame.backdrop[0] == 0.f && frame.backdrop[1] == 0.f && frame.backdrop[2] == 0.f && frame.backdrop[3] == 0.f);
    S.exposure = F.ortho_n ? 1.0f : frame.world.exposure + 0.0f;
    S.out = out_device;
    if (P.bloom) {
        if ((e = sb.bloom_cb.ensure(P.npix)) != hipSuccess || (e = sb.bloom_mips.ensure(bloom_geometry(F.width, F.height).texels)) != hipSuccess)
            return hip_fail(c, "alloc bloom scratch", e);
        S.out = reinterpret_cast<uint32_t *>(sb.bloom_cb.p);
    }
    if ((e = sb.counters.ensure(1)) != hipSuccess) return hip_fail(c, "alloc frame counters", e);
    S.counters = sb.counters.p;
    if (!sb.host_counters) {
        HIP_TRY(c, hipHostMalloc((void **)&sb.host_counters, sizeof(DevCounters), hipHostMallocDefault));
        std::memset(sb.host_counters, 0, sizeof(DevCounters));
    }
    if (!sb.counters_clean) HIP_TRY(c, hipMemsetAsync(sb.counters.p, 0, sizeof(DevCounters), fs.stream));
    sb.counters_clean = false;
    if (P.ordered) {
        if (record_predicts(P, sb, frame)) {
            S.tile_order = sb.tile_order.p;
            S.queue_start = P.n_queues ? sb.queue_start.p : nullptr;
        } else if (P.n_queues) {
            S.tile_order = fs.tile_static.p;
            S.queue_start = fs.queue_static.p;
        }
        if (P.use_feedback) {
            const uint32_t *const before = sb.tile_cost.p;
            if ((e = sb.tile_cost.ensure(n_tiles)) != hipSuccess) return hip_fail(c, "alloc tile feedback", e);
            if (sb.tile_cost.p != before) sb.cost_clean_n = 0;
            if (sb.cost_clean_n < n_tiles) HIP_TRY(c, hipMemsetAsync(sb.tile_cost.p, 0, (size_t)n_tiles * sizeof(uint32_t), fs.stream));
            sb.cost_clean_n = 0;
            S.tile_cost = sb.tile_cost.p;
            std::memcpy(sb.cost_sig, P.sig, sizeof(P.sig));
        }
    }
    if (P.ui) {
        const size_t samples = F.antialias ? 4 : 1;
        if ((e = sb.acc.ensure(samples * P.npix)) != hipSuccess) return hip_fail(c, "alloc accumulators", e);
        S.acc_buf = sb.acc.p;
        if (P.split) {
            if ((e = sb.split_depth.ensure(samples * P.npix)) != hipSuccess) return hip_fail(c, "alloc sample depths", e);
            F.split_depth[j] = sb.split_depth.p;
        }
    }
    F.split_ui_exposure[j] = frame.ui.exposure + 0.0f;
    return AIC_OK;
}

int bind_pixel_edges(aic_ctx *c, aic_ctx::FrameSlot &fs, DevFrame &F, const uint32_t width, const uint32_t height) {
    if (fs.edges_w != width || fs.edges_h != height || !fs.edges.p) {
// ... 583 lines not shown
```

all_is_cubes_amd/csrc/aic_light_bounce.h:

```cpp
#pragma once

#include <hip/hip_runtime.h>
#include <stdint.h>

#include "aic_colour.h"
#include "aic_device.h"
#include "aic_encode.h"
#include "aic_lightmath.h"
#include "aic_raycast.h"

namespace aic {


AIC_DEV int opaque_s(int v) { asm volatile("" : "+s"(v)); return v; }
AIC_DEV uint32_t opaque_s(uint32_t v) { asm volatile("" : "+s"(v)); return v; }
AIC_DEV float opaque_s(float v) { asm volatile("" : "+s"(v)); return v; }
template <class LayerT>
AIC_DEV LightGridView light_view(const LayerT &L) {
    LightGridView G;
    G.light = L.light;
    G.lo_x = opaque_s(L.lo[0]); G.lo_y = opaque_s(L.lo[1]); G.lo_z = opaque_s(L.lo[2]);
    G.size_x = opaque_s(L.size[0]); G.size_y = opaque_s(L.size[1]); G.size_z = opaque_s(L.size[2]);
    G.sky_nx = opaque_s(L.block_sky[0]); G.sky_ny = opaque_s(L.block_sky[1]); G.sky_nz = opaque_s(L.block_sky[2]);
    G.sky_px = opaque_s(L.block_sky[3]); G.sky_py = opaque_s(L.block_sky[4]); G.sky_pz = opaque_s(L.block_sky[5]);
    G.sky_mean = opaque_s(L.block_sky[6]);
    return G;
}

template <bool DIAG, class LayerT>
AIC_DEV uint32_t get_packed_light(const LayerT &L, int cx, int cy, int cz, uint32_t &nlight) {
    if (DIAG) nlight++;
    uint32_t dx = (uint32_t)cx - (uint32_t)L.lo[0];
    uint32_t dy = (uint32_t)cy - (uint32_t)L.lo[1];
    uint32_t dz = (uint32_t)cz - (uint32_t)L.lo[2];
    if ((dx >= (uint32_t)L.size[0]) | (dy >= (uint32_t)L.size[1]) | (dz >= (uint32_t)L.size[2]))
        return lm_light_outside(light_view(L), cx, cy, cz);
    size_t idx = ((size_t)dx * (size_t)L.size[1] + dy) * (size_t)L.size[2] + dz;
    return L.light[idx];
}

struct BounceRng {
    unsigned long long s0, s1, s2, s3;
};
AIC_DEV unsigned long long rotl64(unsigned long long x, int k) { return (x << k) | (x >> (64 - k)); }
AIC_DEV BounceRng bounce_rng_seed(unsigned long long state) {
    unsigned long long w[4];
#pragma unroll
    for (int i = 0; i < 4; i++) {
        state += 0x9e3779b97f4a7c15ull;
        unsigned long long z = state;
        z = (z ^ (z >> 30)) * 0xbf58476d1ce4e5b9ull;
        z = (z ^ (z >> 27)) * 0x94d049bb133111ebull;
        w[i] = z ^ (z >> 31);
    }
    return BounceRng{w[0], w[1], w[2], w[3]};
}
AIC_DEV unsigned long long bounce_rng_next(BounceRng &g) {
    const unsigned long long result = rotl64(g.s0 + g.s3, 23) + g.s0;
    const unsigned long long t = g.s1 << 17;
    g.s2 ^= g.s0;
    g.s3 ^= g.s1;
    g.s1 ^= g.s2;
    g.s0 ^= g.s3;
    g.s2 ^= t;
    g.s3 = rotl64(g.s3, 45);
    return result;
}
AIC_DEV double bounce_uniform_m1_1(BounceRng &g) {
    const double value1_2 = __longlong_as_double((long long)((bounce_rng_next(g) >> 12) | 0x3ff0000000000000ull));
    return (value1_2 - 1.0) * 2.0 + -1.0;
}
AIC_DEV void bounce_unit_sphere(BounceRng &g, double out[3]) {
    for (;;) {
        const double x1 = bounce_uniform_m1_1(g), x2 = bounce_uniform_m1_1(g);
        const double sum = x1 * x1 + x2 * x2;
        if (sum >= 1.0) continue;
        const double factor = 2.0 * sqrt(1.0 - sum);
        out[0] = x1 * factor; out[1] = x2 * factor; out[2] = 1.0 - 2.0 * sum;
        return;
    }
}

struct SecSurface {
    float r, g, b, a, e0, e1, e2;
    int cx, cy, cz, face;
    double t;
};

template <bool DIAG, class LayerT>
AIC_DEV uint32_t bounce_secondary_ray(const LayerT &L, const float *sky_mem, const float *lut, const double *s_pow, bool big,
                                      double ox, double oy, double oz, double dirx, double diry, double dirz, float out[3]) {
    const auto &opt = L.opt;
    const bool vol = opt.transparency == 1;
    const uint32_t idx_mask = big ? 0xffffu : kCubeIndexMask;
    const uint32_t oct = ((dirx >= 0.0) ? 4u : 0u) | ((diry >= 0.0) ? 2u : 0u) | ((dirz >= 0.0) ? 1u : 0u);
    float sky[3];
    {
        const float *p = sky_mem + (L.sky_kind != 0 ? 3u * oct : 0u);
        sky[0] = p[0]; sky[1] = p[1]; sky[2] = p[2];
    }
    const double t_abs = sqrt(dirx * dirx + diry * diry + dirz * dirz);
    const float t_view = (float)(t_abs / opt.view_distance);
    const bool fog_on = opt.fog != 0;
    const float fog_blend = opt.fog == 1 ? 1.0f : (opt.fog == 2 ? 0.5f : 0.0f);
    const RayDir rd = raydir_init(dirx, diry, dirz);
    const double half_over_len = 0.5 / t_abs;
    const int olx = L.lo[0], oly = L.lo[1], olz = L.lo[2], osx = L.size[0], osy = L.size[1], osz = L.size[2];
    const int ohx = olx + osx, ohy = oly + osy, ohz = olz + osz;
    const LvlLim oi = lvl_init(ox, oy, oz, rd, true, olx, oly, olz, ohx, ohy, ohz, true, half_over_len);
    Lvl os = oi.s;
    const Lim ol = oi.lim;
    bool inb = false;
    Lvl is = oi.s;
    Lim il = oi.lim;
    int ilx = 0, ily = 0, ilz = 0, isx = 1, isy = 1, isz = 1, bcx = 0, bcy = 0, bcz = 0;
    uint32_t blk_res = 1u, vox_off = 0u, pal_off = 0u, n_inv = 0u;
    ColorBuf acc;
    acc.l0 = acc.l1 = acc.l2 = 0.f; acc.t = 1.0f;
    uint32_t count = 0;
    bool has_last = false;
    SecSurface last;
    last.r = last.g = last.b = last.a = last.e0 = last.e1 = last.e2 = 0.f; last.cx = last.cy = last.cz = last.face = 0; last.t = 0.0;

    auto count_step_should_stop = [&]() -> bool {
        count++;
        if (count > 1000u) return true;
        return cb_opaque(acc);
    };
    auto through_surface = [&](const SecSurface &sf) {
        float r = sf.r, g = sf.g, b = sf.b, a = sf.a;
        if (opt.transparency == 2) {
            if (a > opt.threshold) a = 1.0f;
            else { r = g = b = a = 0.f; }
        }
        if (a == 0.f && sf.e0 == 0.f && sf.e1 == 0.f && sf.e2 == 0.f) return;
        int nx = 0, ny = 0, nz = 0;
        if (sf.face == 1) nx = -1; else if (sf.face == 2) ny = -1; else if (sf.face == 3) nz = -1;
        else if (sf.face == 4) nx = 1; else if (sf.face == 5) ny = 1; else if (sf.face == 6) nz = 1;
        uint32_t nl = 0;
        const uint32_t txl = get_packed_light<false>(L, sf.cx + nx, sf.cy + ny, sf.cz + nz, nl);
        const float i0 = lut[txl & 255u], i1 = lut[(txl >> 8) & 255u], i2 = lut[(txl >> 16) & 255u];
        float o0 = ps_mul(ps_mul(r, i0), a) + sf.e0, o1 = ps_mul(ps_mul(g, i1), a) + sf.e1, o2 = ps_mul(ps_mul(b, i2), a) + sf.e2;
        float tr = 1.0f - a;
        if (fog_on) {
            float rel = (float)sf.t * t_view;
            rel = rel < 0.0f ? 0.0f : (rel > 1.0f ? 1.0f : rel);
            const float sq = rel * rel;
            const float fog_exp = 1.0f - expf_table(-1.6f * rel, s_pow);
            const float fudged = fog_exp / 0.79810348f;
            const float amount = zo_clamped(fudged * (1.0f - fog_blend) + (sq * sq) * fog_blend);
            const float comp = 1.0f - amount;
            o0 = ps_mul(o0, comp) + ps_mul(sky[0], amount);
            o1 = ps_mul(o1, comp) + ps_mul(sky[1], amount);
            o2 = ps_mul(o2, comp) + ps_mul(sky[2], amount);
            tr *= comp;
        }
        cb_add(acc, o0, o1, o2, tr);
    };
    auto through_span = [&](SecSurface sf, double exit_t) {
        float thickness = (float)((exit_t - sf.t) * t_abs);
        thickness = fmaxf(thickness, 0.0f);
        float coeff;
        if (thickness == 0.0f) {
            if (sf.a == 1.0f) coeff = 1.0f;
            else { sf.r = sf.g = sf.b = sf.a = 0.f; coeff = 0.0f; }
        } else {
            const float unit_t = 1.0f - sf.a;
            float depth_t;
            if (unit_t == 0.0f) depth_t = 0.0f;
            else if (unit_t == 1.0f) depth_t = 1.0f;
            else if (!(thickness < __uint_as_float(0x7f800000u))) depth_t = 0.0f;
            else depth_t = powf_table(unit_t, thickness, s_pow);
            sf.a = zo_clamped(1.0f - depth_t);
            const float ec = (unit_t == 1.0f) ? thickness : (depth_t - 1.f) / (unit_t - 1.f);
            coeff = fmaxf(ec, 0.0f);
        }
        const float c = ps_clamped(coeff);
        sf.e0 = ps_mul(sf.e0, c); sf.e1 = ps_mul(sf.e1, c); sf.e2 = ps_mul(sf.e2, c);
        through_surface(sf);
    };

    for (;;) {
        int kind = 0;
        double t = 0.0;
        SecSurface cur = last;
        if (inb) {
            const NextResult nr = lvl_next(is, il, rd, ilx, ily, ilz, ilx + isx, ily + isy, ilz + isz);
            is = nr.s;
            if (nr.got) {
                const double as = __hiloint2double((int)((1023u - (31u - (uint32_t)__clz((int)blk_res))) << 20), 0);
                t = is.last_t * as;
                kind = 1;
                if (!nr.is_exit) {
                    const uint32_t vi = (uint32_t)(((uint32_t)(is.cx - ilx) * (uint32_t)isy + (uint32_t)(is.cy - ily)) * (uint32_t)isz + (uint32_t)(is.cz - ilz));
                    const uint32_t code = L.pool[(size_t)vox_off + vi];
                    if (code >= n_inv) {
                        const DevPaletteEntry *pe = &L.palette[pal_off + code];
                        kind = 2;
                        cur.r = pe->color[0]; cur.g = pe->color[1]; cur.b = pe->color[2]; cur.a = pe->color[3];
                        cur.e0 = pe->emission[0]; cur.e1 = pe->emission[1]; cur.e2 = pe->emission[2];
                        cur.cx = bcx; cur.cy = bcy; cur.cz = bcz; cur.face = lvl_face(is); cur.t = t;
                    }
                }
            } else {
                inb = false;
            }
        }
        if (kind == 0) {
            const NextResult nr = lvl_next(os, ol, rd, olx, oly, olz, ohx, ohy, ohz);
            os = nr.s;
            if (!nr.got) break;
            t = os.last_t;
            kind = 1;
            if (!nr.is_exit) {
                const size_t ci = ((size_t)(uint32_t)(os.cx - olx) * (size_t)osy + (size_t)(uint32_t)(os.cy - oly)) * (size_t)osz + (size_t)(uint32_t)(os.cz - olz);
                const uint32_t entry = L.pool[ci];
                const uint32_t bi = entry & idx_mask;
                const uint32_t cls = big ? ((L.cls[bi >> 4] >> ((bi & 15u) << 1)) & 3u) : cube_entry_class(entry);
                const DevBlock *tb = &L.blocks[bi];
                if (cls == 1u) {
                    kind = 2;
                    cur.r = tb->color[0]; cur.g = tb->color[1]; cur.b = tb->color[2]; cur.a = tb->color[3];
                    cur.e0 = tb->emission[0]; cur.e1 = tb->emission[1]; cur.e2 = tb->emission[2];
                    cur.cx = os.cx; cur.cy = os.cy; cur.cz = os.cz; cur.face = lvl_face(os); cur.t = t;
                } else if (cls == 2u) {
                    kind = 3;
                    blk_res = tb->kind & 255u;
                    const uint32_t vlo = tb->vlo_packed, vsz = tb->vsize_packed;
                    ilx = (int)(vlo & 255u); ily = (int)((vlo >> 8) & 255u); ilz = (int)((vlo >> 16) & 255u);
                    isx = (int)(vsz & 255u); isy = (int)((vsz >> 8) & 255u); isz = (int)((vsz >> 16) & 255u);
                    vox_off = tb->vox_off; pal_off = tb->pal_off; n_inv = tb->n_invisible;
                    bcx = os.cx; bcy = os.cy; bcz = os.cz;
                    const double kd = (double)blk_res;
                    const LvlLim ii = lvl_init((ox - (double)bcx) * kd, (oy - (double)bcy) * kd, (oz - (double)bcz) * kd, rd, true, ilx, ily, ilz,
                                               ilx + isx, ily + isy, ilz + isz, true, half_over_len);
                    is = ii.s;
                    il = ii.lim;
                    inb = true;
                }
            }
        }
        if (vol) {
            if (count_step_should_stop()) break;
            if (kind == 2) {
                if (has_last) through_span(last, cur.t);
                last = cur;
                has_last = true;
            } else {
                if (has_last) { has_last = false; through_span(last, t); }
                if (kind == 3 && count_step_should_stop()) break;
            }
        } else {
            if (count_step_should_stop()) break;
            if (kind == 2) through_surface(cur);
        }
    }
    cb_add(acc, sky[0] * 1.0f, sky[1] * 1.0f, sky[2] * 1.0f, 0.0f);
    if (opt.debug_pixel_cost) {
        const float n = ps_clamped((float)count);
        const float red = ps_clamped(ps_mul(0.02f, n) * 1.0f);
        const float green = ps_clamped(ps_mul(0.002f, n) * 1.0f);
        float cur_rgba[4];
        cb_to_rgba(acc, cur_rgba);
        const float blue = ps_clamped(luminance(cur_rgba[0], cur_rgba[1], cur_rgba[2]) * 0.2f);
        acc.l0 = red; acc.l1 = green; acc.l2 = blue; acc.t = 0.0f;
    }
    float c[4];
    cb_to_rgba(acc, c);
    out[0] = c[0]; out[1] = c[1]; out[2] = c[2];
    (void)DIAG;
    return count;
}

}
```

all_is_cubes_amd/csrc/aic_trace.hip:

```cpp

#include <hip/hip_runtime.h>
#include <stdint.h>

#include <cstddef>
#include <cstdlib>

#include "aic_device.h"
#include "aic_encode.h"
#include "aic_lightmath.h"
#include "aic_launch.h"
#include "aic_tunables.h"
#include "aic_raycast.h"
#include "aic_colour.h"
#include "aic_light_bounce.h"
#include "aic_scene_kernels.h"
#include "aic_probe_kernels.h"

namespace aic {


AIC_DEV uint32_t wave_popc(unsigned long long m) {
    uint32_t n;
    asm volatile("s_bcnt1_i32_b64 %0, %1" : "=s"(n) : "s"(m) : "scc");
    return n;
// ... 376 lines not shown
                    "s_mov_b64 exec, %[sv]\n\t"
                    : [x0] "+v"(tx), [x1] "+v"(ty), [x2] "+v"(tz), [x3] "+v"(last_t), [x4] "+v"(tdx), [x5] "+v"(tdy), [x6] "+v"(tdz), [sv] "=&s"(sv)
                    : [p] "v"(x_paddr), [m] "s"(x_got)
                    : "memory", "scc");
                asm volatile(
                    "s_and_saveexec_b64 %[sv], %[m]\n\t"
                    "s_cbranch_execz .Lxb%=\n\t"
                    "ds_wrxchg_rtn_b32 %[w0], %[p], %[w0] offset:56\n\t"
                    "ds_wrxchg_rtn_b32 %[w1], %[p], %[w1] offset:60\n\t"
                    "ds_wrxchg_rtn_b32 %[w2], %[p], %[w2] offset:64\n\t"
                    "ds_wrxchg_rtn_b32 %[w3], %[p], %[w3] offset:68\n\t"
                    "ds_wrxchg_rtn_b32 %[w4], %[p], %[w4] offset:72\n\t"
                    "ds_wrxchg_rtn_b32 %[w5], %[p], %[w5] offset:76\n\t"
                    "ds_wrxchg_rtn_b32 %[w6], %[p], %[w6] offset:80\n\t"
                    "ds_wrxchg_rtn_b32 %[w7], %[p], %[w7] offset:84\n\t"
                    "ds_wrxchg_rtn_b32 %[w8], %[p], %[w8] offset:88\n\t"
                    "ds_wrxchg_rtn_b32 %[w9], %[p], %[w9] offset:92\n\t"
                    "ds_wrxchg_rtn_b32 %[wa], %[p], %[wa] offset:96\n\t"
                    "ds_wrxchg_rtn_b32 %[wb], %[p], %[wb] offset:100\n\t"
                    "s_waitcnt lgkmcnt(0)\n"
                    ".Lxb%=:\n\t"
                    "s_mov_b64 exec, %[sv]\n\t"
                    : [w0] "+v"(rx), [w1] "+v"(ry), [w2] "+v"(rz), [w3] "+v"(boff), [w4] "+v"(ssx), [w5] "+v"(ssy), [w6] "+v"(ssz), [w7] "+v"(thr), [w8] "+v"(raw),
                      [w9] "+v"(lax), [wa] "+v"(st), [wb] "+v"(count), [sv] "=&s"(sv)
                    : [p] "v"(x_paddr), [m] "s"(x_got)
                    : "memory", "scc");
                asm volatile(
                    "s_and_saveexec_b64 %[sv], %[m]\n\t"
                    "s_cbranch_execz .Lxc%=\n\t"
                    "ds_wrxchg_rtn_b32 %[w0], %[p], %[w0] offset:104\n\t"
                    "ds_wrxchg_rtn_b32 %[w1], %[p], %[w1] offset:108\n\t"
                    "ds_wrxchg_rtn_b32 %[w2], %[p], %[w2] offset:112\n\t"
                    "ds_wrxchg_rtn_b32 %[w3], %[p], %[w3] offset:116\n\t"
                    "ds_wrxchg_rtn_b32 %[w4], %[p], %[w4] offset:120\n\t"
                    "ds_wrxchg_rtn_b32 %[w5], %[p], %[w5] offset:124\n\t"
                    "ds_wrxchg_rtn_b32 %[w6], %[p], %[w6] offset:128\n\t"
                    "ds_wrxchg_rtn_b32 %[w7], %[p], %[w7] offset:132\n\t"
                    "ds_wrxchg_rtn_b32 %[w8], %[p], %[w8] offset:136\n\t"
                    "ds_wrxchg_rtn_b32 %[w9], %[p], %[w9] offset:140\n\t"
                    "ds_wrxchg_rtn_b32 %[wa], %[p], %[wa] offset:144\n\t"
                    "ds_wrxchg_rtn_b32 %[wb], %[p], %[wb] offset:148\n\t"
                    "ds_wrxchg_rtn_b32 %[wc], %[p], %[wc] offset:152\n\t"
                    "s_waitcnt lgkmcnt(0)\n\t"
                    "s_mov_b64 exec, %[f]\n\t"
                    "v_mov_b32 %[w0], 0xa0\n"
                    ".Lxc%=:\n\t"
                    "s_mov_b64 exec, %[sv]\n\t"
                    : [w0] "+v"(ev), [w1] "+v"(blk_pal_off), [w2] "+v"(blk_geo), [w3] "+v"(blk_vsz), [w4] "+v"(acc.l0), [w5] "+v"(acc.l1), [w6] "+v"(acc.l2), [w7] "+v"(acc.t),
                      [w8] "+v"(pend0), [w9] "+v"(pend1), [wa] "+v"(pend2), [wb] "+v"(pend_tr), [wc] "+v"(col), [sv] "=&s"(sv)
                    : [p] "v"(x_paddr), [m] "s"(x_got), [f] "s"(x_fresh)
                    : "memory", "scc");
                static_assert((EV_NEWRAY | EV_TAKE) == 0xa0u, "the literal in the asm above");
                const bool got = __builtin_amdgcn_inverse_ballot_w64(x_got), fresh = __builtin_amdgcn_inverse_ballot_w64(x_fresh);
                const uint32_t n_picked = wave_popc(x_got & ~x_fresh);
                const uint32_t x_slot = x_slot_tag & 255u, x_tag = x_slot_tag >> 8;
                if (got && x_tag != TAG_FREE) atomicAdd(reinterpret_cast<uint32_t *>(&s_census) + (x_tag - 1u), 1u);
                if (got) __hip_atomic_store(&s_tag[x_slot], x_tag, __ATOMIC_RELEASE, __HIP_MEMORY_SCOPE_WORKGROUP);
                if (lane == 0u && n_picked != 0u) atomicSub(reinterpret_cast<uint32_t *>(&s_census) + (x_want - 1u), n_picked);
                (void)fresh;
                AIC_PROF(31, 1);
                AIC_PROF(32, wave_popc(x_got));
                AIC_PROF(34, n_picked);
                AIC_PROF(35, wave_popc(__builtin_amdgcn_ballot_w64(got && x_tag != TAG_FREE)));
                m_st = __ballot(ev < 4u);
                b_shade = __ballot((ev & EV_SHADE) != 0u);
                b_enter = __ballot((ev & EV_ENTER) != 0u);
                b_ray = __ballot((ev & (EV_FINISH | EV_NEWRAY)) != 0u);
                n_step = (int)wave_popc(m_st);
                c_shade = (int)wave_popc(b_shade); c_enter = (int)wave_popc(b_enter); c_ray = (int)wave_popc(b_ray);
                AIC_TICK(33);
            }
            }
            }
            else { AIC_TICK(19); }
            AIC_SECTION(scheduler_tail);
            if (!settled && (run == 0u ? n_step : (run == EV_SHADE ? c_shade : (run == EV_ENTER ? c_enter : c_ray))) == 0) {
                AIC_PROF(36, 1);
                if (spun_out()) break;
                __builtin_amdgcn_s_sleep(4);
                continue;
            }
        } else {
        if ((m_st | b_shade | b_enter | b_ray) == 0ull) break;
        {
            int best = c_shade;
            uint32_t kind = EV_SHADE;
            if (c_enter > best) { best = c_enter; kind = EV_ENTER; }
            if (c_ray > best) { best = c_ray; kind = EV_FINISH; }
            const int alive = n_step + c_shade + c_enter + c_ray;
            const int part_t = (alive * AIC_FRAC_T) >> 3, part_n = (alive * AIC_FRAC_N) >> 3;
            const int t_lo = opaque_s(part_t > 0 ? part_t : 1);
            const int t_batch = t_lo < AIC_T_BATCH ? t_lo : AIC_T_BATCH;
            const int n_few = part_n < AIC_N_FEW ? part_n : AIC_N_FEW;
            if (best > 0 && (best >= t_batch || n_step <= n_few)) run = kind;
        }
        AIC_TICK(19);
        }
        if (run != 0u) {
            AIC_SECTION(event_prologue);
            typedef const __attribute__((address_space(4))) DevFrame KFrame;
            KFrame *Fq = (KFrame *)__builtin_amdgcn_kernarg_segment_ptr();
            asm volatile("" : "+s"(Fq));
            KFrame &F = *Fq;
            const auto &L = F.layer;
            const auto &opt = L.opt;
            typedef const __attribute__((address_space(4))) DevSub KSub;
            KSub *Sq = reinterpret_cast<KSub *>(reinterpret_cast<const __attribute__((address_space(4))) char *>(Fq) + offsetof(DevFrame, sub)) +
                       (F.n_sub > 1u ? (blockIdx.x & (F.n_sub - 1u)) : 0u);
            asm volatile("" : "+s"(Sq));
            KSub &S = *Sq;
            const bool ui_pass = F.pass == 1;
            const bool include_sky = F.pass == 0;
            const bool fog_on = (opt.fog != 0) && include_sky;
            const size_t npix = (size_t)F.width * F.local_rows;
            const int n_samples = F.antialias ? 4 : 1;
            const int olx = L.lo[0], oly = L.lo[1], olz = L.lo[2];
            const int osx_i = L.size[0], osy_i = L.size[1], osz_i = L.size[2];
            const uint32_t tile_px = F.tile * F.tile;
            const uint32_t macro_shift = (uint32_t)__ffs((int)F.macro) - 1u;
            const uint32_t macro_px_shift = macro_shift + (uint32_t)__ffs((int)F.tile) - 1u;
            const uint32_t n_virtual = (F.macros_x * F.macros_y) << (macro_shift * 2u);
            auto sky_now = [&](float out[3]) {
                if (L.sky_kind != 0) {
                    const float *p = (const float *)((const char *)(const void *)Fq + offsetof(DevFrame, layer) + offsetof(DevLayer, sky)) + 3u * ((st >> 24) & 7u);
                    out[0] = p[0]; out[1] = p[1]; out[2] = p[2];
                } else {
                    out[0] = L.sky[0][0]; out[1] = L.sky[0][1]; out[2] = L.sky[0][2];
                }
            };
            AIC_PROF(0, 1);
            AIC_PROF(1, c_shade + c_enter + c_ray);
#ifdef AIC_TAIL_PROF
            if (__builtin_amdgcn_readfirstlane((int)dry)) { tail_events++; AIC_PROF(30, 1); }
#endif
            AIC_PROF(4, run == EV_SHADE ? 1 : 0); AIC_PROF(5, run == EV_SHADE ? c_shade : 0);
            AIC_PROF(6, run == EV_ENTER ? 1 : 0); AIC_PROF(7, run == EV_ENTER ? c_enter : 0);
            AIC_PROF(8, run == EV_FINISH ? 1 : 0); AIC_PROF(9, run == EV_FINISH ? c_ray : 0);
            auto ray_of_pixel = [&](const uint32_t x, const uint32_t lrow, const int sample, const bool want_dir, double o[3], double dir[3]) -> bool {
                const uint32_t mode = F.ray_mode;
                if (mode <= 1u) {
                    const double *const ex = F.edge_x, *const ey = F.edge_y;
                    uint32_t y = lrow;
                    if (mode == 1u) {
                        const uint32_t srows = opaque_s(F.strip_rows);
                        const uint32_t strip = lrow / srows;
                        y = (F.part + strip * F.n_parts) * srows + (lrow - strip * srows);
                    }
                    const double x0 = ex[x], x1 = ex[x + 1u], y0 = ey[y], y1 = ey[y + 1u];
                    double px, py;
                    if (n_samples == 4) {
                        const double ux = (sample == 0) ? 1. / 8. : (sample == 1) ? 3. / 8. : (sample == 2) ? 5. / 8. : 7. / 8.;
                        const double uy = (sample == 0) ? 5. / 8. : (sample == 1) ? 1. / 8. : (sample == 2) ? 7. / 8. : 3. / 8.;
                        px = x0 + (x1 - x0) * ux;
                        py = y0 + (y1 - y0) * uy;
                    } else {
                        px = (x0 + x1) / 2.0;
                        py = (y0 + y1) / 2.0;
                    }
                    unproject(S.inv, px, py, 0.0, o);
                    if (want_dir) {
                        double f[3];
                        unproject(S.inv, px, py, 1.0, f);
                        dir[0] = f[0] - o[0]; dir[1] = f[1] - o[1]; dir[2] = f[2] - o[2];
                    }
                    return true;
                }
                const size_t pix = (size_t)lrow * F.width + x;
                if (F.rays) {
                    const double2 *const r = reinterpret_cast<const double2 *>(F.rays + 6u * pix);
                    const double2 r0 = r[0], r1 = r[1];
                    o[0] = r0.x; o[1] = r0.y; o[2] = r1.x;
                    if (want_dir) {
                        const double2 r2 = r[2];
                        dir[0] = r1.y; dir[1] = r2.x; dir[2] = r2.y;
                    }
                    return true;
                }
                uint32_t y = lrow;
                if (F.n_parts > 1u) {
                    const uint32_t srows = opaque_s(F.strip_rows);
                    const uint32_t strip = lrow / srows;
                    y = (F.part + strip * F.n_parts) * srows + (lrow - strip * srows);
                }
                const bool listed = DIAG && F.pixels;
                uint32_t gx = x;
                if (listed) {
                    const uint32_t p_ = F.pixels[pix], pw_ = opaque_s(F.px_width);
                    y = p_ / pw_;
                    gx = p_ - y * pw_;
                }
                double px, py;
                if (F.pixel_centers) {
                    const uint32_t fw = opaque_s(listed ? F.px_width : F.width), fh = opaque_s(listed ? F.px_height : F.height);
                    px = ((double)gx + 0.5) / (double)fw * 2.0 - 1.0;
                    py = -(((double)y + 0.5) / (double)fh * 2.0 - 1.0);
                } else {
                    double x0, x1, y0, y1;
                    if (F.patches) {
                        const double *r = F.patches + 4u * pix;
                        x0 = r[0]; y0 = r[1]; x1 = r[2]; y1 = r[3];
                    } else if (F.edge_x) {
                        x0 = F.edge_x[gx]; x1 = F.edge_x[gx + 1u]; y0 = F.edge_y[y]; y1 = F.edge_y[y + 1u];
                    } else {
                        const uint32_t fw = opaque_s(F.width), fh = opaque_s(F.height);
                        x0 = fb_x_edge(fw, gx); x1 = fb_x_edge(fw, gx + 1);
                        y0 = fb_y_edge(fh, y); y1 = fb_y_edge(fh, y + 1);
                    }
                    if (n_samples == 4) {
                        const double ux = (sample == 0) ? 1. / 8. : (sample == 1) ? 3. / 8. : (sample == 2) ? 5. / 8. : 7. / 8.;
                        const double uy = (sample == 0) ? 5. / 8. : (sample == 1) ? 1. / 8. : (sample == 2) ? 7. / 8. : 3. / 8.;
                        px = x0 + (x1 - x0) * ux;
                        py = y0 + (y1 - y0) * uy;
                    } else {
                        px = (x0 + x1) / 2.0;
                        py = (y0 + y1) / 2.0;
                    }
                }
                bool have_ray = L.present != 0;
                o[0] = o[1] = o[2] = 0.0;
                if (want_dir) dir[0] = dir[1] = dir[2] = 0.0;
                if (have_ray && F.ortho_n) {
                    int vsel = -1;
                    for (int v = 0; v < F.ortho_n; v++) {
                        const uint32_t vx = F.ortho[v].x0, vy = F.ortho[v].y0, vw = F.ortho[v].w, vh = F.ortho[v].h;
                        if (vsel < 0 && gx >= vx && y >= vy && gx - vx < vw && y - vy < vh) vsel = v;
                    }
                    have_ray = false;
                    if (vsel >= 0) {
                        const DevOrthoView *V = &F.ortho[vsel];
                        double p[3];
                        unproject(V->m, (double)(gx - V->x0), (double)(y - V->y0), 0.0, p);
                        int cube[3];
                        if (cube_containing(p, cube)) {
                            have_ray = true;
                            for (int a = 0; a < 3; a++) {
                                o[a] = (double)cube[a] + (double)(float)(p[a] - (double)cube[a]);
                                if (want_dir) dir[a] = V->dir[a];
                            }
                        }
                    }
                } else if (have_ray) {
                    unproject(S.inv, px, py, 0.0, o);
                    if (want_dir) {
                        double f[3];
                        unproject(S.inv, px, py, 1.0, f);
                        dir[0] = f[0] - o[0]; dir[1] = f[1] - o[1]; dir[2] = f[2] - o[2];
                    }
                }
                return have_ray;
            };
            char *const cold_wg = XCHG ? reinterpret_cast<char *>(F.ray_cold) + (size_t)blockIdx.x * (size_t)(NCOL * 16u) : nullptr;
            auto off32 = [&](uint32_t k) -> uint32_t { return (k * NCOL + col) * 4u; };
            auto cold_origin = [&](double &ox, double &oy, double &oz) {
                if constexpr (XCHG) {
                    const uint32_t pxy_ = c32[K_PXY][col];
                    double o_[3];
                    (void)ray_of_pixel(pxy_ & 0xffffu, pxy_ >> 16, (int)((st >> 14) & 3u), false, o_, nullptr);
                    ox = o_[0]; oy = o_[1]; oz = o_[2];
                } else {
                    ox = c64[XCHG ? 0 : (int)C_OX][col]; oy = c64[XCHG ? 0 : (int)C_OY][col]; oz = c64[XCHG ? 0 : (int)C_OZ][col];
                }
            };
            auto cold_direction = [&](double &dx, double &dy, double &dz) { dx = c64[C_DX][col]; dy = c64[C_DY][col]; dz = c64[C_DZ][col]; };
            auto cold_sums_load = [&](float v[4]) {
                if constexpr (XCHG) {
                    for (uint32_t k = 0; k < 4u; k++) v[k] = __uint_as_float(__hip_atomic_load(reinterpret_cast<uint32_t *>(cold_wg + off32(k)), __ATOMIC_RELAXED, __HIP_MEMORY_SCOPE_WORKGROUP));
                } else {
                    v[0] = __uint_as_float(c32[XCHG ? 0 : (int)K_S0][col]); v[1] = __uint_as_float(c32[XCHG ? 0 : (int)K_S1][col]);
                    v[2] = __uint_as_float(c32[XCHG ? 0 : (int)K_S2][col]); v[3] = __uint_as_float(c32[XCHG ? 0 : (int)K_ST][col]);
                }
            };
            auto cold_sums_store = [&](float v0, float v1, float v2, float v3) {
                if constexpr (XCHG) {
                    *reinterpret_cast<float *>(cold_wg + off32(0u)) = v0; *reinterpret_cast<float *>(cold_wg + off32(1u)) = v1;
                    *reinterpret_cast<float *>(cold_wg + off32(2u)) = v2; *reinterpret_cast<float *>(cold_wg + off32(3u)) = v3;
                    asm volatile("s_waitcnt vmcnt(0)" ::: "memory");
                } else {
                    c32[XCHG ? 0 : (int)K_S0][col] = __float_as_uint(v0); c32[XCHG ? 0 : (int)K_S1][col] = __float_as_uint(v1);
                    c32[XCHG ? 0 : (int)K_S2][col] = __float_as_uint(v2); c32[XCHG ? 0 : (int)K_ST][col] = __float_as_uint(v3);
                }
            };
            const uint32_t posx = (st >> 26) & 1u, posy = (st >> 25) & 1u, posz = (st >> 24) & 1u;
            if (run == EV_SHADE) {
            AIC_SECTION(shade_geometry);
            if (ev & EV_SHADE) {
                const bool inb = (st & ST_IN_BLOCK) != 0;
                const uint32_t blk_res = 1u << (blk_geo >> 24), blk_vlo = blk_geo & 0xffffffu;
                const double as = inb ? __hiloint2double((int)((1023u - (blk_geo >> 24)) << 20), 0) : 1.0;
                const double t_enter = last_t * as;
                const uint32_t s_rx = c32[K_SRX][col], s_ry = c32[K_SRY][col], s_rz = c32[K_SRZ][col];
                const int ocx = coord(posx, osx_i, inb ? s_rx : rx) + olx, ocy = coord(posy, osy_i, inb ? s_ry : ry) + oly,
                          ocz = coord(posz, osz_i, inb ? s_rz : rz) + olz;
                Lvl ca;
                ca.tx = tx; ca.ty = ty; ca.tz = tz; ca.last_t = last_t; ca.st = face_now() << 2;
                if (inb) {
                    ca.cx = coord(posx, (int)(blk_vsz & 255u), rx) + (int)(blk_vlo & 255u);
                    ca.cy = coord(posy, (int)((blk_vsz >> 8) & 255u), ry) + (int)((blk_vlo >> 8) & 255u);
                    ca.cz = coord(posz, (int)((blk_vsz >> 16) & 255u), rz) + (int)((blk_vlo >> 16) & 255u);
                } else {
                    ca.cx = ocx; ca.cy = ocy; ca.cz = ocz;
                }
                const uint32_t shade_ref = inb ? (blk_pal_off + raw) : (0x80000000u | (raw & idx_mask));
                static_assert(offsetof(DevBlock, color) == 0 && offsetof(DevBlock, emission) == 16 && offsetof(DevPaletteEntry, color) == 0 && offsetof(DevPaletteEntry, emission) == 16, "one record layout");
                const char *const rec_p = (shade_ref & 0x80000000u) ? reinterpret_cast<const char *>(&L.blocks[shade_ref & 0xffffu]) : reinterpret_cast<const char *>(&L.palette[shade_ref]);
                const float4 rec_col = *reinterpret_cast<const float4 *>(rec_p);
                const float4 rec_em = *reinterpret_cast<const float4 *>(rec_p + 16);
                float i0 = 1.0f, i1 = 1.0f, i2 = 1.0f;
                uint32_t nl = 0;
                double ip[3] = {0.0, 0.0, 0.0};
                AIC_SECTION(shade_light);
                if (LMODE != 0) {
                    const int face = lvl_face(ca);
                    if (LMODE == 1 || LMODE == 3) {
                        int nx = 0, ny = 0, nz = 0;
                        if (face == 1) nx = -1; else if (face == 2) ny = -1; else if (face == 3) nz = -1;
                        else if (face == 4) nx = 1; else if (face == 5) ny = 1; else if (face == 6) nz = 1;
                        const uint32_t txl = get_packed_light<DIAG>(L, ocx + nx, ocy + ny, ocz + nz, nl);
                        i0 = lut[txl & 255u]; i1 = lut[(txl >> 8) & 255u]; i2 = lut[(txl >> 16) & 255u];
                    }
                    if (LMODE >= 2) {
                        double ox = 0.0, oy = 0.0, oz = 0.0, dx, dy, dz;
                        cold_direction(dx, dy, dz);
                        const bool need_o = (face == FACE_WITHIN) | (dx == 0.0) | (dy == 0.0) | (dz == 0.0);
                        if (__ballot(need_o) != 0ull) {
                            if (need_o) {
                                cold_origin(ox, oy, oz);
                                if (inb) {
                                    const double kd = (double)blk_res;
                                    ox = (ox - (double)ocx) * kd; oy = (oy - (double)ocy) * kd; oz = (oz - (double)ocz) * kd;
                                }
                            }
                        }
                        double vp[3];
                        intersection_point(ca, ox, oy, oz, dx, dy, dz, vp);
                        ip[0] = inb ? vp[0] * as + (double)ocx : vp[0];
                        ip[1] = inb ? vp[1] * as + (double)ocy : vp[1];
                        ip[2] = inb ? vp[2] * as + (double)ocz : vp[2];
                    }
                    if (LMODE == 2) {
                        float fin[4];
                        lm_interpolated_light(light_view(L), lut, ocx, ocy, ocz, ip[0], ip[1], ip[2], face, opt.lighting, fin, DIAG ? &nl : nullptr);
                        const float w = fmaxf(fin[3], 0.1f);
                        if (__ballot(w != 1.0f) == 0ull) {
                            i0 = fin[0]; i1 = fin[1]; i2 = fin[2];
                        } else {
                            const float r0 = __builtin_amdgcn_rcpf(w);
                            const float rr = __builtin_fmaf(__builtin_fmaf(-w, r0, 1.0f), r0, r0);
                            auto quot = [&](const float x) -> float {
                                float q = x * rr;
                                q = __builtin_fmaf(__builtin_fmaf(-w, q, x), rr, q);
                                return __builtin_fmaf(__builtin_fmaf(-w, q, x), rr, q);
                            };
                            i0 = quot(fin[0]); i1 = quot(fin[1]); i2 = quot(fin[2]);
                        }
                    }
                }
                AIC_TICK(18);
                AIC_SECTION(shade_colour_span);
                float r = rec_col.x, g = rec_col.y, b = rec_col.z, a = rec_col.w, e0 = rec_em.x, e1 = rec_em.y, e2 = rec_em.z;
                bool will_flush = true;
                if (VOL) {
                    double t_exit = 0.0;
                    if (!(ev & EV_DEAD)) {
                        const int pk = pick_axis(tx, ty, tz);
                        t_exit = (pk == 0 ? tx : (pk == 1 ? ty : tz)) * as;
                    } else if (inb && (st & ST_OUTER_ALIVE)) {
                        const double s_tx = c64[C_STX][col], s_ty = c64[C_STY][col], s_tz = c64[C_STZ][col];
                        const int pk = pick_axis(s_tx, s_ty, s_tz);
                        t_exit = pk == 0 ? s_tx : (pk == 1 ? s_ty : s_tz);
                    } else {
                        will_flush = false;
                    }
                    float thickness = (float)((t_exit - t_enter) * c64[C_TABS][col]);
                    thickness = fmaxf(thickness, 0.0f);
                    float coeff;
                    if (thickness == 0.0f) {
                        if (a == 1.0f) coeff = 1.0f;
                        else { r = g = b = a = 0.f; coeff = 0.0f; }
                    } else {
                        const float unit_t = 1.0f - a;
                        float depth_t;
                        if (unit_t == 0.0f) depth_t = 0.0f;
                        else if (unit_t == 1.0f) depth_t = 1.0f;
                        else if (!(thickness < __uint_as_float(0x7f800000u))) depth_t = 0.0f;
                        else depth_t = powf_table(unit_t, thickness, s_pow);
                        a = zo_clamped(1.0f - depth_t);
                        const float ec = (unit_t == 1.0f) ? thickness : (depth_t - 1.f) / (unit_t - 1.f);
                        coeff = fmaxf(ec, 0.0f);
                    }
                    const float c = ps_clamped(coeff);
                    e0 = ps_mul(e0, c); e1 = ps_mul(e1, c); e2 = ps_mul(e2, c);
                }
                AIC_SECTION(shade_to_light_fog);
                if (opt.transparency == 2) {
                    if (a > opt.threshold) a = 1.0f;
                    else { r = g = b = a = 0.f; }
                }
                if (LMODE == 3 && a == 1.0f && (!VOL || (will_flush && count <= 999u))) {
                    const int face = lvl_face(ca);
                    double nvx = 0.0, nvy = 0.0, nvz = 0.0;
                    if (face == 1) nvx = -1.0; else if (face == 2) nvy = -1.0; else if (face == 3) nvz = -1.0;
                    else if (face == 4) nvx = 1.0; else if (face == 5) nvy = 1.0; else if (face == 6) nvz = 1.0;
                    const float *sky_mem = (const float *)((const char *)(const void *)Fq + offsetof(DevFrame, layer) + offsetof(DevLayer, sky));
                    const uint32_t n_samples_b = (uint32_t)opt.bounce_samples & 255u;
                    float m0 = 0.f, m1 = 0.f, m2 = 0.f;
                    for (uint32_t k = 0; k < n_samples_b; k++) {
                        double u[3];
                        bounce_unit_sphere(brng, u);
                        float c3[3];
                        sec_steps += bounce_secondary_ray<DIAG>(L, sky_mem, lut, s_pow, BIG, ip[0] + nvx * 0.0001, ip[1] + nvy * 0.0001, ip[2] + nvz * 0.0001,
                                                                nvx + u[0], nvy + u[1], nvz + u[2], c3);
                        m0 += c3[0]; m1 += c3[1]; m2 += c3[2];
                    }
                    const float kk = ps_clamped(1.0f / (float)n_samples_b);
                    i0 = ps_mul(m0, kk); i1 = ps_mul(m1, kk); i2 = ps_mul(m2, kk);
                    nl = 0;
                }
                float o0 = 0.f, o1 = 0.f, o2 = 0.f, tr = 1.0f;
                const bool visible = !(a == 0.f && e0 == 0.f && e1 == 0.f && e2 == 0.f);
                if (visible) {
                    o0 = ps_mul(ps_mul(r, i0), a) + e0;
                    o1 = ps_mul(ps_mul(g, i1), a) + e1;
                    o2 = ps_mul(ps_mul(b, i2), a) + e2;
                    tr = 1.0f - a;
                    if (fog_on) {
                        float sky[3];
                        sky_now(sky);
                        const float fog_blend = opt.fog == 1 ? 1.0f : (opt.fog == 2 ? 0.5f : 0.0f);
                        float rel = (float)t_enter * __uint_as_float(c32[K_TVIEW][col]);
                        rel = rel < 0.0f ? 0.0f : (rel > 1.0f ? 1.0f : rel);
                        const float sq = rel * rel;
                        float amount;
                        if (opt.fog == 1) {
                            amount = zo_clamped((sq * sq) * 1.0f);
                        } else {
                            const float fog_exp = 1.0f - expf_table(-1.6f * rel, s_pow);
                            const float fudged = fog_exp / 0.79810348f;
                            amount = zo_clamped(fudged * (1.0f - fog_blend) + (sq * sq) * fog_blend);
                        }
                        const float comp = 1.0f - amount;
                        o0 = ps_mul(o0, comp) + ps_mul(sky[0], amount);
                        o1 = ps_mul(o1, comp) + ps_mul(sky[1], amount);
                        o2 = ps_mul(o2, comp) + ps_mul(sky[2], amount);
                        tr *= comp;
                    }
                }
                AIC_SECTION(shade_apply);
                SurfDiag sd;
                if (DIAG) {
                    sd.nlight = nl;
                    sd.cube[0] = ocx; sd.cube[1] = ocy; sd.cube[2] = ocz;
                    if (inb) {
                        sd.voxel[0] = ca.cx; sd.voxel[1] = ca.cy; sd.voxel[2] = ca.cz;
                        sd.res = (int)blk_res; sd.block = (int)c32[XCHG ? 0 : (int)K_BLK][col];
                    } else {
                        sd.voxel[0] = sd.voxel[1] = sd.voxel[2] = 0;
                        sd.res = 1; sd.block = (int)(shade_ref & 0xffffu);
                    }
                    sd.face = lvl_face(ca);
                }
                if (VOL) {
                    if (will_flush) {
                        bool early = !DIAG && !(ev & EV_DEAD) && count <= 999u;
                        const float n0 = acc.l0 + o0 * acc.t, n1 = acc.l1 + o1 * acc.t, n2 = acc.l2 + o2 * acc.t, nt = acc.t * tr;
                        early = early && !(nt < 1.0f / 256.0f);
                        const bool finish_now = !DIAG && !(ev & EV_DEAD) && count <= 998u && (nt < 1.0f / 256.0f);
                        if (finish_now) {
                            const int pk = pick_axis(tx, ty, tz);
                            const uint32_t r_next = pk == 0 ? rx : (pk == 1 ? ry : rz);
                            const bool second = (r_next != 0u) || (inb && (st & ST_OUTER_ALIVE));
                            acc.l0 = n0; acc.l1 = n1; acc.l2 = n2; acc.t = nt;
                            count += second ? 2u : 1u;
                            st |= ST_OPAQUE;
                            ev = (ev & EV_SHADE) | EV_FINISH;
                        } else if (early) {
                            acc.l0 = n0; acc.l1 = n1; acc.l2 = n2; acc.t = nt;
                        } else {
                            pend0 = o0; pend1 = o1; pend2 = o2; pend_tr = tr;
                            st |= ST_HAS_LAST;
                        }
                        if (DIAG) { pend_d = sd; pend_t = t_enter; pend_visible = visible; }
                    }
                } else if (visible) {
                    cb_add(acc, o0, o1, o2, tr);
                    if (cb_opaque(acc)) {
                        st |= ST_OPAQUE;
                        if (!DIAG && !(ev & EV_DEAD) && count <= 999u) {
                            count += 1u;
                            ev = (ev & EV_SHADE) | EV_FINISH;
                        }
                    }
                    if (DIAG) {
                        dg.n_hits++;
                        dg.n_light += sd.nlight;
                        sp_smp = fmin(sp_smp, t_enter);
                        split_layer_after_add(F.hit_layer ? SPLIT_UI : SPLIT_WORLD);
                        if (!dg.hit) {
                            dg.hit = 1;
                            dg.layer = F.hit_layer;
                            for (int a2 = 0; a2 < 3; a2++) { dg.cube[a2] = sd.cube[a2]; dg.voxel[a2] = sd.voxel[a2]; }
                            dg.res = sd.res; dg.face = sd.face; dg.block = sd.block; dg.t = t_enter;
                        }
                    }
                }
                ev &= ~EV_SHADE;
            }
            AIC_SECTION(shade_end);
            } else if (run == EV_ENTER) {
            AIC_SECTION(enter);
            if (ev & EV_ENTER) {
                const uint32_t blk_index = raw & idx_mask;
                if (DIAG) c32[XCHG ? 0 : (int)K_BLK][col] = blk_index;
                const DevBlock *tb = &L.blocks[blk_index];
                const uint32_t blk_res = tb->kind & 255u;
                const uint32_t blk_vlo = tb->vlo_packed;
                blk_geo = ((31u - (uint32_t)__clz((int)blk_res)) << 24) | blk_vlo;
                blk_vsz = tb->vsize_packed;
                blk_pal_off = tb->pal_off;
                double ox, oy, oz, edx, edy, edz;
                cold_origin(ox, oy, oz);
                cold_direction(edx, edy, edz);
                const uint32_t n_invisible = tb->n_invisible;
                const uint32_t vox_off = tb->vox_off;
                const double kd = (double)blk_res;
                const int acx = coord(posx, osx_i, rx) + olx, acy = coord(posy, osy_i, ry) + oly, acz = coord(posz, osz_i, rz) + olz;
                const double sx_ = (ox - (double)acx) * kd, sy_ = (oy - (double)acy) * kd, sz_ = (oz - (double)acz) * kd;
                c64[C_STX][col] = tx; c64[C_STY][col] = ty; c64[C_STZ][col] = tz;
                c32[K_SRX][col] = rx; c32[K_SRY][col] = ry; c32[K_SRZ][col] = rz; c32[K_SBOFF][col] = boff;
                st = (st & ~((7u << 16) | ST_OUTER_ALIVE)) | (face_now() << 16) | ((ev & EV_DEAD) ? 0u : ST_OUTER_ALIVE);
                const int ilx = (int)(blk_vlo & 255u), ily = (int)((blk_vlo >> 8) & 255u), ilz = (int)((blk_vlo >> 16) & 255u);
                const int isx = (int)(blk_vsz & 255u), isy = (int)((blk_vsz >> 8) & 255u), isz = (int)((blk_vsz >> 16) & 255u);
                const RayDir rd = make_rd(edx, edy, edz);
                const LvlLim ll = lvl_init(sx_, sy_, sz_, rd, true, ilx, ily, ilz, ilx + isx, ily + isy, ilz + isz, true, 0.5 / c64[C_TABS][col]);
                const FirstCube f = lvl_first_masks(ll.s, rd, ilx, ily, ilz, ilx + isx, ily + isy, ilz + isz);
                const int vcx = f.cx - ilx, vcy = f.cy - ily, vcz = f.cz - ilz;
                boff = 2u * (vox_off + (uint32_t)(((uint32_t)vcx * (uint32_t)isy + (uint32_t)vcy) * (uint32_t)isz + (uint32_t)vcz));
                constexpr bool first_lookup = !DIAG && !BIG;
                const bool first_elig = first_lookup && f.got && f.inbounds && !(st & (ST_HAS_LAST | ST_OPAQUE)) && count <= 999u;
                uint32_t first_raw = 0u;
                if constexpr (first_lookup) { AIC_ISSUE_FIRST_LOOKUP(first_elig, first_raw); }
                tx = f.tx; ty = f.ty; tz = f.tz; last_t = f.last_t;
                rx = posx ? (uint32_t)(isx - 1 - vcx) : (uint32_t)vcx;
                ry = posy ? (uint32_t)(isy - 1 - vcy) : (uint32_t)vcy;
                rz = posz ? (uint32_t)(isz - 1 - vcz) : (uint32_t)vcz;
                ssx = posx ? 2 * isy * isz : -2 * isy * isz; ssy = posy ? 2 * isz : -2 * isz; ssz = posz ? 2 : -2;
                thr = n_invisible;
                lax = f.lax;
                st |= ST_IN_BLOCK;
                bool first_invisible = false;
                if constexpr (first_lookup) {
                    AIC_WAIT_LOOKUP(first_raw);
                    first_invisible = first_elig && first_raw < thr;
                    count += first_invisible ? 1u : 0u;
                }
                ev = ((f.got && !first_invisible) ? EV_FRESH : 0u) | (f.inbounds ? 0u : EV_DEAD);
            }
            AIC_SECTION(enter_end);
            } else {
            AIC_SECTION(finish);
            uint32_t pxy = 0;
            int sample = 0;
            bool want = false;
            if (run == EV_FINISH) {
                pxy = c32[K_PXY][col];
                sample = (ev & EV_TAKE) ? 0 : (int)((st >> 14) & 3u);
            }
            if (run == EV_FINISH && (ev & EV_FINISH)) {
                if (st & ST_TRACED) {
                    if (include_sky) {
                        float sky[3];
                        sky_now(sky);
                        cb_add(acc, sky[0] * 1.0f, sky[1] * 1.0f, sky[2] * 1.0f, 0.0f);
                    } else {
                        cb_add(acc, 0.f, 0.f, 0.f, 1.0f);
                    }
                    if (opt.debug_pixel_cost) {
                        const float n = ps_clamped((float)count);
                        const float red = ps_clamped(ps_mul(0.02f, n) * 1.0f);
                        const float green = ps_clamped(ps_mul(0.002f, n) * 1.0f);
                        float cur_rgba[4];
                        cb_to_rgba(acc, cur_rgba);
                        const float blue = ps_clamped(luminance(cur_rgba[0], cur_rgba[1], cur_rgba[2]) * 0.2f);
                        acc.l0 = red; acc.l1 = green; acc.l2 = blue; acc.t = 0.0f;
                    }
                    { uint32_t t_ = threadIdx.x; asm volatile("" : "+v"(t_)); s_steps[t_] += count + (LMODE == 3 ? sec_steps : 0u); }
#ifdef AIC_PROFILE
                    { const uint32_t dur_ = (uint32_t)__builtin_readcyclecounter() - s_ray_t0[col];
                      if (dur_ > ray_dur_max) { ray_dur_max = dur_; ray_dur_steps = count; } }
#endif
                    if (DIAG) {
                        px_steps += count + (LMODE == 3 ? sec_steps : 0u);
                        split_layer_after_add(F.hit_layer ? SPLIT_UI : SPLIT_WORLD);
                    }
                }
                const uint32_t x = pxy & 0xffffu, lrow = pxy >> 16;
                float aa_sum[4] = {0.f, 0.f, 0.f, 0.f};
                if (S.tile_cost && count > 48u) {
                    uint32_t *tc = &S.tile_cost[(lrow >> macro_px_shift) * F.macros_x + (x >> macro_px_shift)];
                    if (count > *tc) atomicMax(tc, count);
                }
                const size_t pix = (size_t)lrow * F.width + x;
                if (ui_pass) {
                    S.acc_buf[(size_t)sample * npix + pix] = make_float4(acc.l0, acc.l1, acc.l2, acc.t);
                    if (DIAG) {
                        double *const sd_ = F.split_depth[F.n_sub > 1u ? (blockIdx.x & (F.n_sub - 1u)) : 0u];
                        if (sd_) sd_[(size_t)sample * npix + pix] = sp_smp;
                    }
                } else {
                    if (!F.bare_trace && !cb_opaque(acc)) {
                        acc.l0 = 0.f + (NO_WORLD_TO_SHOW * 1.0f) * 1.0f;
                        acc.l1 = acc.l0;
                        acc.l2 = acc.l0;
                        acc.t = 1.0f * (1.0f - 1.0f);
                        if (DIAG) {
                            sp_smp = __longlong_as_double(0x7ff0000000000000LL);
                            sp_lay = (sp_lay & ~3u) | SPLIT_WORLD;
                        }
                    }
                    if (DIAG) {
                        sp_px = fmin(sp_px, sp_smp);
                        if (!(sp_lay & 12u)) sp_lay |= (sp_lay & 3u) << 2;
                    }
                    if (n_samples == 4) {
                        cold_sums_load(aa_sum);
                        aa_sum[0] += acc.l0; aa_sum[1] += acc.l1; aa_sum[2] += acc.l2; aa_sum[3] += acc.t;
                        if (sample < 3) cold_sums_store(aa_sum[0], aa_sum[1], aa_sum[2], aa_sum[3]);
                    }
                }
                sample++;
                if (sample < n_samples) {
                    ev = EV_NEWRAY;
                } else {
                    if (!ui_pass) {
                        ColorBuf pixel;
                        if (n_samples == 4) {
                            pixel.l0 = aa_sum[0] / 4.0f; pixel.l1 = aa_sum[1] / 4.0f; pixel.l2 = aa_sum[2] / 4.0f; pixel.t = aa_sum[3] / 4.0f;
                        } else {
                            pixel = acc;
                        }
                        float c[4];
                        cb_to_rgba(pixel, c);
                        size_t opix = pix, depth_plane = npix * 8u;
                        if (DIAG && F.pixels) {
                            if (F.px_in_place) { opix = F.pixels[pix]; depth_plane = (size_t)F.px_width * F.px_height * 8u; }
                            else depth_plane = (size_t)F.n_patches * 8u;
                        }
                        if (DIAG && F.out_mode == 3) {
                            const uint32_t sub_ = F.n_sub > 1u ? (blockIdx.x & (F.n_sub - 1u)) : 0u;
                            const uint32_t pl = (sp_lay >> 2) & 3u;
                            const float e = pl == SPLIT_UI ? F.split_ui_exposure[sub_] : (pl == SPLIT_WORLD ? S.exposure : 1.0f);
                            float a = 1.0f - pixel.t;
                            a = a < 0.0f ? 0.0f : a;
                            a = a > 1.0f ? 1.0f : a;
                            auto f16_bits = [](float v) -> uint32_t { return (uint32_t)__builtin_bit_cast(uint16_t, (_Float16)v); };
                            reinterpret_cast<uint2 *>(S.out)[opix] =
                                make_uint2(f16_bits(pixel.l0 * e) | (f16_bits(pixel.l1 * e) << 16), f16_bits(pixel.l2 * e) | (f16_bits(a) << 16));
                            double d = sp_px;
                            d = d < 0.0 ? 0.0 : d;
                            d = d > 1.0 ? 1.0 : d;
                            const double z_ = ((0.0 * 0.0 + 0.0 * 0.0) + d * F.depth_zw[0]) + F.depth_zw[1];
                            const double w_ = ((0.0 * 0.0 + 0.0 * 0.0) + d * F.depth_zw[2]) + F.depth_zw[3];
                            const float layer_factor = pl == SPLIT_WORLD ? 1.0f : -1.0f;
                            reinterpret_cast<float *>(reinterpret_cast<char *>(S.out) + depth_plane)[opix] = (float)(z_ / w_) * layer_factor;
                        } else if (F.out_mode != 0) {
                            reinterpret_cast<float4 *>(S.out)[opix] =
                                F.out_mode == 1 ? make_float4(c[0], c[1], c[2], c[3]) : make_float4(pixel.l0, pixel.l1, pixel.l2, pixel.t);
                        } else {
                        const float ex = S.exposure;
                        float r = ps_mul(c[0], ex), g = ps_mul(c[1], ex), bl = ps_mul(c[2], ex);
                        const float m = F.maximum_intensity;
                        if (isfinite(m)) {
                            if (F.tone_mapping == 0) {
                                r = r < 0.f ? 0.f : (r > m ? m : r);
                                g = g < 0.f ? 0.f : (g > m ? m : g);
                                bl = bl < 0.f ? 0.f : (bl > m ? m : bl);
                            } else {
                                const float scale = ps_clamped(1.0f / (1.0f + luminance(r, g, bl) / m));
                                r = ps_mul(r, scale); g = ps_mul(g, scale); bl = ps_mul(bl, scale);
                            }
                        }
                        uint32_t R, G, B;
                        srgb8_rgb_bucket(r, g, bl, F.srgb_buckets, R, G, B);
                        const uint32_t A = round_sat_u8(c[3] * 255.0f);
                        S.out[opix] = R | (G << 8) | (B << 16) | (A << 24);
                        }
                    }
                    if (DIAG) {
                        if (F.aux) {
                            DevAux &a = F.aux[pix];
                            a.hit = dg.hit & 1;
// ... 624 lines not shown
```

all_is_cubes_amd/csrc/aic_tunables.h:

```cpp
#pragma once

#ifndef AIC_MIN_WAVES
#define AIC_MIN_WAVES 4
#endif
#ifndef AIC_WG_THREADS
#define AIC_WG_THREADS 256
#endif

#ifndef AIC_T_BATCH
#define AIC_T_BATCH 32
#endif
#ifndef AIC_N_FEW
#define AIC_N_FEW 24
#endif
#ifndef AIC_FRAC_T
#define AIC_FRAC_T 4
#endif
#ifndef AIC_FRAC_N
#define AIC_FRAC_N 3
#endif

#ifndef AIC_STEP_REPS
#define AIC_STEP_REPS 2
#endif
#ifndef AIC_FAST_STEPS
#define AIC_FAST_STEPS 16
#endif
#ifndef AIC_FAST_MIN
#define AIC_FAST_MIN 16
#endif

#ifndef AIC_BONUS_MIN
#define AIC_BONUS_MIN 1
#endif

#ifndef AIC_XWG_THREADS
#define AIC_XWG_THREADS 256
#endif
#ifndef AIC_POOL
#define AIC_POOL (AIC_XWG_THREADS >= 512 ? 160 : 64)
#endif
#ifndef AIC_XCHG_FULL
#define AIC_XCHG_FULL 48
#endif
#ifndef AIC_XCHG_MIN_GAIN
#define AIC_XCHG_MIN_GAIN 8
#endif
#ifndef AIC_XCHG_PARK_MIN
#define AIC_XCHG_PARK_MIN 8
#endif

#ifndef AIC_REPROJECT_RATIO_CAP
#define AIC_REPROJECT_RATIO_CAP 8.0f
#endif
```

Measured before the change: 6581.

## Precompute per-material log2 and reciprocal for transparent volume shading

Adds a per-block and per-palette-entry material table holding log2(1-alpha) and 1/(unit_t-1), computed on the host at upload time and kept in sync through compaction and block updates. The volume shading path loads this record and skips the log2 half of the table-based pow and the float divide, using a branchless exp2 and a reciprocal-based division. It also selects the block or palette record pointer arithmetically instead of through a branch. In exchange it adds an extra 16-byte load per shaded sample, extra device memory, and host-side work on scene upload.

```diff
diff --git a/all_is_cubes_amd/csrc/aic_abi.cpp b/all_is_cubes_amd/csrc/aic_abi.cpp
--- a/all_is_cubes_amd/csrc/aic_abi.cpp
+++ b/all_is_cubes_amd/csrc/aic_abi.cpp
@@ -128,6 +128,8 @@
     std::memcpy(&bits, &v, sizeof(bits));
     return bits == 0u || bits == 0x3f800000u;
 }
+
+constexpr uint64_t kMaxPaletteEntries = 0xfffffff0ull - kMaterialPaletteBase;
 
 int convert_block(aic_ctx *c, const aic_block_desc &d, const uint16_t *voxels, const float *palette, uint32_t vox_off,
                   uint32_t pal_off, DevBlock *out, std::vector<uint16_t> *vox_out, std::vector<DevPaletteEntry> *pal_out) {
@@ -202,6 +204,22 @@
     out->pal_off = pal_off;
     out->n_invisible = n_inv;
     out->pad[0] = block_selectable ? kBlockSelectable : 0u;
+    return AIC_OK;
+}
+
+int write_materials(aic_ctx *c, Layer &l, size_t pal_total, bool keep, const DevBlock *blocks, size_t nb, size_t b0, const DevPaletteEntry *pal, size_t np,
+                    size_t p0) {
+    hipError_t e;
+    if ((e = l.material.ensure((size_t)kMaterialPaletteBase + pal_total, keep, c->stream)) != hipSuccess) return hip_fail(c, "alloc materials", e);
+    std::vector<DevMaterial> m(nb > np ? nb : np);
+    if (nb) {
+        for (size_t i = 0; i < nb; i++) m[i] = material_entry((blocks[i].kind & 255u) == 0u ? blocks[i].color[3] : 0.0f);
+        HIP_TRY(c, hipMemcpy(l.material.p + b0, m.data(), nb * sizeof(DevMaterial), hipMemcpyHostToDevice));
+    }
+    if (np) {
+        for (size_t i = 0; i < np; i++) m[i] = material_entry(pal[i].color[3]);
+        HIP_TRY(c, hipMemcpy(l.material.p + kMaterialPaletteBase + p0, m.data(), np * sizeof(DevMaterial), hipMemcpyHostToDevice));
+    }
     return AIC_OK;
 }
 
@@ -383,7 +401,7 @@
         size_t nvox = one ? 1 : (size_t)(d.vsize[0] > 0 ? d.vsize[0] : 0) * (size_t)(d.vsize[1] > 0 ? d.vsize[1] : 0) * (size_t)(d.vsize[2] > 0 ? d.vsize[2] : 0);
         if ((uint64_t)d.vox_off + nvox > s->n_voxels || (uint64_t)d.pal_off + d.pal_len > s->n_palette)
             return fail(c, AIC_ERR_INVALID, "block voxel/palette range exceeds the pools");
-        if (n + vox.size() + nvox > kMaxPoolElems || pal.size() + d.pal_len > 0xfffffff0ull) return fail(c, AIC_ERR_INVALID, "pool too large");
+        if (n + vox.size() + nvox > kMaxPoolElems || pal.size() + d.pal_len > kMaxPaletteEntries) return fail(c, AIC_ERR_INVALID, "pool too large");
         const size_t vb = vox.size(), pb = pal.size();
         int rc = convert_block(c, d, s->voxels ? s->voxels + d.vox_off : nullptr, s->palette ? s->palette + 8 * (size_t)d.pal_off : nullptr,
                                (uint32_t)(n + vox.size()), (uint32_t)pal.size(), &blocks[i], &vox, &pal);
@@ -419,6 +437,7 @@
         launch_open_cubes(l.pool.p, s->size, c->stream);
     }
     if (!pal.empty()) HIP_TRY(c, hipMemcpyAsync(l.palette.p, pal.data(), pal.size() * sizeof(DevPaletteEntry), hipMemcpyHostToDevice, c->stream));
+    { const int rc = write_materials(c, l, pal.size(), false, blocks.data(), blocks.size(), 0, pal.data(), pal.size(), 0); if (rc != AIC_OK) return rc; }
     HIP_TRY(c, hipStreamSynchronize(c->stream));
 
     for (int a = 0; a < 3; a++) { l.lo[a] = s->lo[a]; l.size[a] = s->size[a]; }
@@ -535,13 +554,16 @@
     for (size_t i = 0; i < l.host_blocks.size(); i++) { need_vox += l.vox_cap[i]; need_pal += l.pal_cap[i]; }
     DevBuf<uint16_t> np;
     DevBuf<DevPaletteEntry> npal;
+    DevBuf<DevMaterial> nmat;
     hipError_t e;
     if ((e = np.ensure((size_t)need_vox)) != hipSuccess) return hip_fail(c, "compact pool", e);
     if ((e = npal.ensure((size_t)(need_pal ? need_pal : 1))) != hipSuccess) { np.release(); return hip_fail(c, "compact palette", e); }
+    if ((e = nmat.ensure((size_t)kMaterialPaletteBase + (size_t)(need_pal ? need_pal : 1))) != hipSuccess) { np.release(); npal.release(); return hip_fail(c, "compact materials", e); }
     std::vector<DevBlock> blocks = l.host_blocks;
     std::vector<uint32_t> vbase = l.vox_base, pbase = l.pal_base;
     uint64_t vo = n, po = 0;
     e = n ? hipMemcpyAsync(np.p, l.pool.p, n * sizeof(uint16_t), hipMemcpyDeviceToDevice, c->stream) : hipSuccess;
+    if (e == hipSuccess && !blocks.empty()) e = hipMemcpyAsync(nmat.p, l.material.p, blocks.size() * sizeof(DevMaterial), hipMemcpyDeviceToDevice, c->stream);
     for (size_t i = 0; e == hipSuccess && i < blocks.size(); i++) {
         DevBlock &b = blocks[i];
         if (l.vox_cap[i]) {
@@ -552,6 +574,9 @@
         }
         if (e == hipSuccess && l.pal_cap[i]) {
             e = hipMemcpyAsync(npal.p + po, l.palette.p + l.pal_base[i], (size_t)l.pal_cap[i] * sizeof(DevPaletteEntry), hipMemcpyDeviceToDevice, c->stream);
+            if (e == hipSuccess)
+                e = hipMemcpyAsync(nmat.p + kMaterialPaletteBase + po, l.material.p + kMaterialPaletteBase + l.pal_base[i], (size_t)l.pal_cap[i] * sizeof(DevMaterial),
+                                   hipMemcpyDeviceToDevice, c->stream);
             if ((b.kind & 255u) != 0u) b.pal_off = (uint32_t)po;
             pbase[i] = (uint32_t)po;
             po += l.pal_cap[i];
@@ -564,12 +589,15 @@
         if (!l.host_blocks.empty()) (void)hipMemcpy(l.blocks.p, l.host_blocks.data(), l.host_blocks.size() * sizeof(DevBlock), hipMemcpyHostToDevice);
         np.release();
         npal.release();
+        nmat.release();
         return hip_fail(c, "compact pools", e);
     }
     l.pool.release();
     l.palette.release();
     l.pool = np;
     l.palette = npal;
+    l.material.release();
+    l.material = nmat;
     l.pool.n = (size_t)vo;
     l.palette.n = (size_t)po;
     l.host_blocks.swap(blocks);
@@ -598,7 +626,7 @@
     } else {
         vox_off = (uint32_t)l.pool.n;
         pal_off = (uint32_t)l.palette.n;
-        if ((uint64_t)vox_off + vox.size() > kMaxPoolElems || (uint64_t)pal_off + pal.size() > 0xfffffff0ull)
+        if ((uint64_t)vox_off + vox.size() > kMaxPoolElems || (uint64_t)pal_off + pal.size() > kMaxPaletteEntries)
             return fail(c, AIC_ERR_INVALID, "voxel pool too large");
         if (!vox.empty() && (e = l.pool.ensure(vox_off + vox.size(), true, c->stream)) != hipSuccess) return hip_fail(c, "grow pool", e);
         if (!pal.empty() && (e = l.palette.ensure(pal_off + pal.size(), true, c->stream)) != hipSuccess) return hip_fail(c, "grow palette", e);
@@ -612,6 +640,7 @@
         db.pal_off = pal_off;
         HIP_TRY(c, hipMemcpy(l.palette.p + pal_off, pal.data(), pal.size() * sizeof(DevPaletteEntry), hipMemcpyHostToDevice));
     }
+    { const int mrc = write_materials(c, l, l.palette.n, true, &db, 1, index, pal.data(), pal.size(), pal_off); if (mrc != AIC_OK) return mrc; }
     bool class_changed = false;
     if (!exists) {
         l.host_blocks.push_back(db);
diff --git a/all_is_cubes_amd/csrc/aic_colour.h b/all_is_cubes_amd/csrc/aic_colour.h
--- a/all_is_cubes_amd/csrc/aic_colour.h
+++ b/all_is_cubes_amd/csrc/aic_colour.h
@@ -4,6 +4,7 @@
 #include <stdint.h>
 
 #include "aic_encode.h"
+#include "aic_material.h"
 
 namespace aic {
 
@@ -14,26 +15,8 @@
     return 1.f;
 }
 
-__device__ const double kPowLog2Tab[16][2] = {
-    {0x1.661ec79f8f3bep+0, -0x1.efec65b963019p-2}, {0x1.571ed4aaf883dp+0, -0x1.b0b6832d4fca4p-2},
-    {0x1.49539f0f010bp+0, -0x1.7418b0a1fb77bp-2},  {0x1.3c995b0b80385p+0, -0x1.39de91a6dcf7bp-2},
-    {0x1.30d190c8864a5p+0, -0x1.01d9bf3f2b631p-2}, {0x1.25e227b0b8eap+0, -0x1.97c1d1b3b7afp-3},
-    {0x1.1bb4a4a1a343fp+0, -0x1.2f9e393af3c9fp-3}, {0x1.12358f08ae5bap+0, -0x1.960cbbf788d5cp-4},
-    {0x1.0953f419900a7p+0, -0x1.a6f9db6475fcep-5}, {0x1p+0, 0x0p+0},
-    {0x1.e608cfd9a47acp-1, 0x1.338ca9f24f53dp-4},  {0x1.ca4b31f026aap-1, 0x1.476a9543891bap-3},
-    {0x1.b2036576afce6p-1, 0x1.e840b4ac4e4d2p-3},  {0x1.9c2d163a1aa2dp-1, 0x1.40645f0c6651cp-2},
-    {0x1.886e6037841edp-1, 0x1.88e9c2c1b9ff8p-2},  {0x1.767dcf5534862p-1, 0x1.ce0a44eb17bccp-2},
-};
-__device__ const unsigned long long kPowExp2Tab[32] = {
-    0x3ff0000000000000ull, 0x3fefd9b0d3158574ull, 0x3fefb5586cf9890full, 0x3fef9301d0125b51ull,
-    0x3fef72b83c7d517bull, 0x3fef54873168b9aaull, 0x3fef387a6e756238ull, 0x3fef1e9df51fdee1ull,
-    0x3fef06fe0a31b715ull, 0x3feef1a7373aa9cbull, 0x3feedea64c123422ull, 0x3feece086061892dull,
-    0x3feebfdad5362a27ull, 0x3feeb42b569d4f82ull, 0x3feeab07dd485429ull, 0x3feea47eb03a5585ull,
-    0x3feea09e667f3bcdull, 0x3fee9f75e8ec5f74ull, 0x3feea11473eb0187ull, 0x3feea589994cce13ull,
-    0x3feeace5422aa0dbull, 0x3feeb737b0cdc5e5ull, 0x3feec49182a3f090ull, 0x3feed503b23e255dull,
-    0x3feee89f995ad3adull, 0x3feeff76f2fb5e47ull, 0x3fef199bdd85529cull, 0x3fef3720dcef9069ull,
-    0x3fef5818dcfba487ull, 0x3fef7c97337b9b5full, 0x3fefa4afa2a490daull, 0x3fefd0765b6e4540ull,
-};
+__device__ const double kPowLog2Tab[16][2] = {AIC_POW_LOG2_TAB_INIT};
+__device__ const unsigned long long kPowExp2Tab[32] = {AIC_POW_EXP2_TAB_INIT};
 AIC_DEV void pow_tables_to_lds(double *s_pow, uint32_t tid, uint32_t nthreads) {
     for (uint32_t i = tid; i < 64u; i += nthreads)
         s_pow[i] = i < 32u ? kPowLog2Tab[i >> 1][i & 1u] : __longlong_as_double((long long)kPowExp2Tab[i - 32u]);
@@ -41,41 +24,6 @@
 AIC_DEV bool powf_table_domain(float x, float y) {
     const uint32_t ix = __float_as_uint(x), iy = __float_as_uint(y);
     return ix >= 0x00800000u && ix < 0x3f800000u && iy > 0u && iy < 0x7f800000u;
-}
-AIC_DEV double KC(double v) { asm volatile("" : "+s"(v)); return v; }
-AIC_DEV float powf_table(float x, float y, const double *s_pow) {
-    const uint32_t ix = __float_as_uint(x);
-    const uint32_t tmp = ix - 0x3f330000u;
-    const uint32_t i = (tmp >> 19) & 15u;
-    const uint32_t top = tmp & 0xff800000u;
-    const uint32_t iz = ix - top;
-    const int k = (int)top >> 23;
-    const double invc = s_pow[2u * i], logc = s_pow[2u * i + 1u];
-    const double z = (double)__uint_as_float(iz);
-    const double r = fma(z, invc, -1.0);
-    const double y0 = logc + (double)k;
-    const double r2 = r * r;
-    double yy = fma(KC(0x1.27616c9496e0bp-2), r, KC(-0x1.71969a075c67ap-2));
-    const double pp = fma(KC(0x1.ec70a6ca7baddp-2), r, KC(-0x1.7154748bef6c8p-1));
-    const double r4 = r2 * r2;
-    double q = fma(KC(0x1.71547652ab82bp+0), r, y0);
-    q = fma(pp, r2, q);
-    yy = fma(yy, r4, q);
-    const double ylogx = (double)y * yy;
-    if (ylogx <= -150.0) return 0.0f;
-    double kd = ylogx + KC(0x1.8p+47);
-    const unsigned long long ki = (unsigned long long)__double_as_longlong(kd);
-    kd -= KC(0x1.8p+47);
-    const double rr = ylogx - kd;
-    unsigned long long t = (unsigned long long)__double_as_longlong(s_pow[32u + (uint32_t)(ki & 31u)]);
-    t += ki << 47;
-    const double sc = __longlong_as_double((long long)t);
-    const double zz = fma(KC(0x1.c6af84b912394p-5), rr, KC(0x1.ebfce50fac4f3p-3));
-    const double rr2 = rr * rr;
-    double e = fma(KC(0x1.62e42ff0c52d6p-1), rr, 1.0);
-    e = fma(zz, rr2, e);
-    e = e * sc;
-    return (float)e;
 }
 AIC_DEV float expf_table(float x, const double *s_pow) {
     const double z = KC(0x1.71547652b82fep+5) * (double)x;
diff --git a/all_is_cubes_amd/csrc/aic_ctx.h b/all_is_cubes_amd/csrc/aic_ctx.h
--- a/all_is_cubes_amd/csrc/aic_ctx.h
+++ b/all_is_cubes_amd/csrc/aic_ctx.h
@@ -64,6 +64,7 @@
     DevBuf<uint32_t> light_spare[kLightSpares];
     DevBuf<DevBlock> blocks;
     DevBuf<DevPaletteEntry> palette;
+    DevBuf<DevMaterial> material;
     std::vector<DevBlock> host_blocks;
     std::vector<uint32_t> vox_cap, pal_cap, vox_base, pal_base;
     uint64_t garbage_vox = 0, garbage_pal = 0;
@@ -81,7 +82,7 @@
     uint64_t visible_version = ~0ull;
     size_t n_cubes() const { return (size_t)size[0] * (size_t)size[1] * (size_t)size[2]; }
     void release() {
-        pool.release(); cls.release(); light.release(); blocks.release(); palette.release(); visible_bits.release();
+        pool.release(); cls.release(); light.release(); blocks.release(); palette.release(); material.release(); visible_bits.release();
         visible_version = ~0ull;
         for (auto &sp : light_spare) sp.release();
         host_blocks.clear(); host_cls.clear(); vox_cap.clear(); pal_cap.clear(); vox_base.clear(); pal_base.clear();
diff --git a/all_is_cubes_amd/csrc/aic_device.h b/all_is_cubes_amd/csrc/aic_device.h
--- a/all_is_cubes_amd/csrc/aic_device.h
+++ b/all_is_cubes_amd/csrc/aic_device.h
@@ -2,6 +2,8 @@
 
 #include <hip/hip_runtime.h>
 #include <stdint.h>
+
+#include "aic_material.h"
 
 namespace aic {
 
@@ -46,6 +48,7 @@
     const uint32_t *light;
     const DevBlock *blocks;
     const DevPaletteEntry *palette;
+    const DevMaterial *material;
     int32_t lo[3];
     int32_t size[3];
     uint32_t n_blocks;
diff --git a/all_is_cubes_amd/csrc/aic_frame.cpp b/all_is_cubes_amd/csrc/aic_frame.cpp
--- a/all_is_cubes_amd/csrc/aic_frame.cpp
+++ b/all_is_cubes_amd/csrc/aic_frame.cpp
@@ -28,6 +28,7 @@
     d->light = l.light.p;
     d->blocks = l.blocks.p;
     d->palette = l.palette.p;
+    d->material = l.material.p;
     for (int a = 0; a < 3; a++) { d->lo[a] = l.lo[a]; d->size[a] = l.size[a]; }
     d->air_index = l.air_index;
     d->sky_kind = l.sky_kind;
diff --git a/all_is_cubes_amd/csrc/aic_light_bounce.h b/all_is_cubes_amd/csrc/aic_light_bounce.h
--- a/all_is_cubes_amd/csrc/aic_light_bounce.h
+++ b/all_is_cubes_amd/csrc/aic_light_bounce.h
@@ -84,6 +84,7 @@
 struct SecSurface {
     float r, g, b, a, e0, e1, e2;
     int cx, cy, cz, face;
+    uint32_t mat;
     double t;
 };
 
@@ -120,7 +121,7 @@
     uint32_t count = 0;
     bool has_last = false;
     SecSurface last;
-    last.r = last.g = last.b = last.a = last.e0 = last.e1 = last.e2 = 0.f; last.cx = last.cy = last.cz = last.face = 0; last.t = 0.0;
+    last.r = last.g = last.b = last.a = last.e0 = last.e1 = last.e2 = 0.f; last.cx = last.cy = last.cz = last.face = 0; last.mat = 0u; last.t = 0.0;
 
     auto count_step_should_stop = [&]() -> bool {
         count++;
@@ -170,9 +171,17 @@
             if (unit_t == 0.0f) depth_t = 0.0f;
             else if (unit_t == 1.0f) depth_t = 1.0f;
             else if (!(thickness < __uint_as_float(0x7f800000u))) depth_t = 0.0f;
+#if AIC_MATERIAL_LOG2
+            else depth_t = powf_from_log2(L.material[sf.mat].log2_unit_t, thickness, s_pow);
+#else
             else depth_t = powf_table(unit_t, thickness, s_pow);
+#endif
             sf.a = zo_clamped(1.0f - depth_t);
+#if AIC_MATERIAL_RCP
+            const float ec = (unit_t == 1.0f) ? thickness : div_by_rcp(depth_t - 1.f, unit_t - 1.f, L.material[sf.mat].rcp_um1);
+#else
             const float ec = (unit_t == 1.0f) ? thickness : (depth_t - 1.f) / (unit_t - 1.f);
+#endif
             coeff = fmaxf(ec, 0.0f);
         }
         const float c = ps_clamped(coeff);
@@ -199,7 +208,7 @@
                         kind = 2;
                         cur.r = pe->color[0]; cur.g = pe->color[1]; cur.b = pe->color[2]; cur.a = pe->color[3];
                         cur.e0 = pe->emission[0]; cur.e1 = pe->emission[1]; cur.e2 = pe->emission[2];
-                        cur.cx = bcx; cur.cy = bcy; cur.cz = bcz; cur.face = lvl_face(is); cur.t = t;
+                        cur.cx = bcx; cur.cy = bcy; cur.cz = bcz; cur.face = lvl_face(is); cur.t = t; cur.mat = kMaterialPaletteBase + pal_off + code;
                     }
                 }
             } else {
@@ -222,7 +231,7 @@
                     kind = 2;
                     cur.r = tb->color[0]; cur.g = tb->color[1]; cur.b = tb->color[2]; cur.a = tb->color[3];
                     cur.e0 = tb->emission[0]; cur.e1 = tb->emission[1]; cur.e2 = tb->emission[2];
-                    cur.cx = os.cx; cur.cy = os.cy; cur.cz = os.cz; cur.face = lvl_face(os); cur.t = t;
+                    cur.cx = os.cx; cur.cy = os.cy; cur.cz = os.cz; cur.face = lvl_face(os); cur.t = t; cur.mat = bi;
                 } else if (cls == 2u) {
                     kind = 3;
                     blk_res = tb->kind & 255u;
diff --git a/all_is_cubes_amd/csrc/aic_material.h b/all_is_cubes_amd/csrc/aic_material.h
--- /dev/null
+++ b/all_is_cubes_amd/csrc/aic_material.h
@@ -0,0 +1,138 @@
+#pragma once
+
+#include <math.h>
+#include <stdint.h>
+#include <string.h>
+
+#if defined(__HIPCC__)
+#define AIC_MT_HD __host__ __device__ __forceinline__
+#else
+#define AIC_MT_HD static inline
+#endif
+
+namespace aic {
+
+struct DevMaterial {
+    double log2_unit_t;
+    float rcp_um1;
+    uint32_t pad;
+};
+static_assert(sizeof(DevMaterial) == 16, "a material entry is one 16-byte load");
+static constexpr uint32_t kMaterialPaletteBase = 65536u;
+
+#define AIC_POW_LOG2_TAB_INIT                                                                          \
+    {0x1.661ec79f8f3bep+0, -0x1.efec65b963019p-2}, {0x1.571ed4aaf883dp+0, -0x1.b0b6832d4fca4p-2},      \
+    {0x1.49539f0f010bp+0, -0x1.7418b0a1fb77bp-2},  {0x1.3c995b0b80385p+0, -0x1.39de91a6dcf7bp-2},      \
+    {0x1.30d190c8864a5p+0, -0x1.01d9bf3f2b631p-2}, {0x1.25e227b0b8eap+0, -0x1.97c1d1b3b7afp-3},        \
+    {0x1.1bb4a4a1a343fp+0, -0x1.2f9e393af3c9fp-3}, {0x1.12358f08ae5bap+0, -0x1.960cbbf788d5cp-4},      \
+    {0x1.0953f419900a7p+0, -0x1.a6f9db6475fcep-5}, {0x1p+0, 0x0p+0},                                   \
+    {0x1.e608cfd9a47acp-1, 0x1.338ca9f24f53dp-4},  {0x1.ca4b31f026aap-1, 0x1.476a9543891bap-3},        \
+    {0x1.b2036576afce6p-1, 0x1.e840b4ac4e4d2p-3},  {0x1.9c2d163a1aa2dp-1, 0x1.40645f0c6651cp-2},       \
+    {0x1.886e6037841edp-1, 0x1.88e9c2c1b9ff8p-2},  {0x1.767dcf5534862p-1, 0x1.ce0a44eb17bccp-2}
+#define AIC_POW_EXP2_TAB_INIT                                                                          \
+    0x3ff0000000000000ull, 0x3fefd9b0d3158574ull, 0x3fefb5586cf9890full, 0x3fef9301d0125b51ull,        \
+    0x3fef72b83c7d517bull, 0x3fef54873168b9aaull, 0x3fef387a6e756238ull, 0x3fef1e9df51fdee1ull,        \
+    0x3fef06fe0a31b715ull, 0x3feef1a7373aa9cbull, 0x3feedea64c123422ull, 0x3feece086061892dull,        \
+    0x3feebfdad5362a27ull, 0x3feeb42b569d4f82ull, 0x3feeab07dd485429ull, 0x3feea47eb03a5585ull,        \
+    0x3feea09e667f3bcdull, 0x3fee9f75e8ec5f74ull, 0x3feea11473eb0187ull, 0x3feea589994cce13ull,        \
+    0x3feeace5422aa0dbull, 0x3feeb737b0cdc5e5ull, 0x3feec49182a3f090ull, 0x3feed503b23e255dull,        \
+    0x3feee89f995ad3adull, 0x3feeff76f2fb5e47ull, 0x3fef199bdd85529cull, 0x3fef3720dcef9069ull,        \
+    0x3fef5818dcfba487ull, 0x3fef7c97337b9b5full, 0x3fefa4afa2a490daull, 0x3fefd0765b6e4540ull
+
+AIC_MT_HD uint32_t mt_f2u(float v) { uint32_t u; memcpy(&u, &v, 4); return u; }
+AIC_MT_HD float mt_u2f(uint32_t u) { float v; memcpy(&v, &u, 4); return v; }
+AIC_MT_HD unsigned long long mt_d2u(double v) { unsigned long long u; memcpy(&u, &v, 8); return u; }
+AIC_MT_HD double mt_u2d(unsigned long long u) { double v; memcpy(&v, &u, 8); return v; }
+
+#if defined(__HIP_DEVICE_COMPILE__)
+AIC_MT_HD double KC(double v) { asm volatile("" : "+s"(v)); return v; }
+#else
+AIC_MT_HD double KC(double v) { return v; }
+#endif
+
+
+AIC_MT_HD double pow_log2(float x, const double *s_pow) {
+    const uint32_t ix = mt_f2u(x);
+    const uint32_t tmp = ix - 0x3f330000u;
+    const uint32_t i = (tmp >> 19) & 15u;
+    const uint32_t top = tmp & 0xff800000u;
+    const uint32_t iz = ix - top;
+    const int k = (int)top >> 23;
+    const double invc = s_pow[2u * i], logc = s_pow[2u * i + 1u];
+    const double z = (double)mt_u2f(iz);
+    const double r = __builtin_fma(z, invc, -1.0);
+    const double y0 = logc + (double)k;
+    const double r2 = r * r;
+    double yy = __builtin_fma(KC(0x1.27616c9496e0bp-2), r, KC(-0x1.71969a075c67ap-2));
+    const double pp = __builtin_fma(KC(0x1.ec70a6ca7baddp-2), r, KC(-0x1.7154748bef6c8p-1));
+    const double r4 = r2 * r2;
+    double q = __builtin_fma(KC(0x1.71547652ab82bp+0), r, y0);
+    q = __builtin_fma(pp, r2, q);
+    yy = __builtin_fma(yy, r4, q);
+    return yy;
+}
+AIC_MT_HD float powf_from_log2(double yy, float y, const double *s_pow) {
+    const double ylogx = (double)y * yy;
+    if (ylogx <= -150.0) return 0.0f;
+    double kd = ylogx + KC(0x1.8p+47);
+    const unsigned long long ki = mt_d2u(kd);
+    kd -= KC(0x1.8p+47);
+    const double rr = ylogx - kd;
+    unsigned long long t = mt_d2u(s_pow[32u + (uint32_t)(ki & 31u)]);
+    t += ki << 47;
+    const double sc = mt_u2d(t);
+    const double zz = __builtin_fma(KC(0x1.c6af84b912394p-5), rr, KC(0x1.ebfce50fac4f3p-3));
+    const double rr2 = rr * rr;
+    double e = __builtin_fma(KC(0x1.62e42ff0c52d6p-1), rr, 1.0);
+    e = __builtin_fma(zz, rr2, e);
+    e = e * sc;
+    return (float)e;
+}
+AIC_MT_HD float powf_from_log2_select(double yy, float y, const double *s_pow) {
+    const double ylogx = (double)y * yy;
+    double kd = ylogx + KC(0x1.8p+47);
+    const unsigned long long ki = mt_d2u(kd);
+    kd -= KC(0x1.8p+47);
+    const double rr = ylogx - kd;
+    unsigned long long t = mt_d2u(s_pow[32u + (uint32_t)(ki & 31u)]);
+    t += ki << 47;
+    const double sc = mt_u2d(t);
+    const double zz = __builtin_fma(KC(0x1.c6af84b912394p-5), rr, KC(0x1.ebfce50fac4f3p-3));
+    const double rr2 = rr * rr;
+    double e = __builtin_fma(KC(0x1.62e42ff0c52d6p-1), rr, 1.0);
+    e = __builtin_fma(zz, rr2, e);
+    e = e * sc;
+    const float ef = (float)e;
+    return ylogx <= -150.0 ? 0.0f : ef;
+}
+AIC_MT_HD float powf_table(float x, float y, const double *s_pow) { return powf_from_log2(pow_log2(x, s_pow), y, s_pow); }
+
+AIC_MT_HD float div_by_rcp(float a, float b, float y) {
+    const float q0 = a * y;
+    const float q1 = __builtin_fmaf(__builtin_fmaf(-b, q0, a), y, q0);
+    return __builtin_fmaf(__builtin_fmaf(-b, q1, a), y, q1);
+}
+
+struct PowTablesHost {
+    double s_pow[64];
+    PowTablesHost() {
+        const double log2_tab[16][2] = {AIC_POW_LOG2_TAB_INIT};
+        const unsigned long long exp2_tab[32] = {AIC_POW_EXP2_TAB_INIT};
+        for (uint32_t i = 0; i < 64u; i++) s_pow[i] = i < 32u ? log2_tab[i >> 1][i & 1u] : mt_u2d(exp2_tab[i - 32u]);
+    }
+};
+static inline const double *pow_tables_host() {
+    static const PowTablesHost t;
+    return t.s_pow;
+}
+static inline DevMaterial material_of_unit_t(float unit_t) {
+    DevMaterial m;
+    m.log2_unit_t = 0.0; m.rcp_um1 = 0.0f; m.pad = 0u;
+    if (unit_t >= 1.17549435e-38f && unit_t < 1.0f) m.log2_unit_t = pow_log2(unit_t, pow_tables_host());
+    else if (unit_t < 1.0f) m.log2_unit_t = -HUGE_VAL;
+    if (unit_t < 1.0f) m.rcp_um1 = 1.0f / (unit_t - 1.0f);
+    return m;
+}
+static inline DevMaterial material_entry(float alpha) { return material_of_unit_t(1.0f - alpha); }
+
+}
diff --git a/all_is_cubes_amd/csrc/aic_trace.hip b/all_is_cubes_amd/csrc/aic_trace.hip
--- a/all_is_cubes_amd/csrc/aic_trace.hip
+++ b/all_is_cubes_amd/csrc/aic_trace.hip
@@ -702,9 +702,22 @@
                 }
                 const uint32_t shade_ref = inb ? (blk_pal_off + raw) : (0x80000000u | (raw & idx_mask));
                 static_assert(offsetof(DevBlock, color) == 0 && offsetof(DevBlock, emission) == 16 && offsetof(DevPaletteEntry, color) == 0 && offsetof(DevPaletteEntry, emission) == 16, "one record layout");
+#if AIC_REC_SELECT
+                const char *blocks_p = reinterpret_cast<const char *>(L.blocks), *palette_p = reinterpret_cast<const char *>(L.palette);
+                asm volatile("" : "+s"(blocks_p), "+s"(palette_p));
+                const bool rec_blk = (shade_ref & 0x80000000u) != 0u;
+                const char *const rec_p = (rec_blk ? blocks_p : palette_p) + ((uint64_t)(rec_blk ? (shade_ref & 0xffffu) << 1 : shade_ref) << 5);
+#else
                 const char *const rec_p = (shade_ref & 0x80000000u) ? reinterpret_cast<const char *>(&L.blocks[shade_ref & 0xffffu]) : reinterpret_cast<const char *>(&L.palette[shade_ref]);
+#endif
                 const float4 rec_col = *reinterpret_cast<const float4 *>(rec_p);
                 const float4 rec_em = *reinterpret_cast<const float4 *>(rec_p + 16);
+                float4 rec_mat = make_float4(0.f, 0.f, 0.f, 0.f);
+                if (VOL && (AIC_MATERIAL_LOG2 || AIC_MATERIAL_RCP)) {
+                    const uint32_t mat_ref = (shade_ref & 0x80000000u) ? (shade_ref & 0xffffu) : kMaterialPaletteBase + shade_ref;
+                    static_assert(offsetof(DevMaterial, log2_unit_t) == 0 && offsetof(DevMaterial, rcp_um1) == 8, "x, y: the logarithm's halves; z: the reciprocal");
+                    rec_mat = *reinterpret_cast<const float4 *>(&L.material[mat_ref]);
+                }
                 float i0 = 1.0f, i1 = 1.0f, i2 = 1.0f;
                 uint32_t nl = 0;
                 double ip[3] = {0.0, 0.0, 0.0};
@@ -780,12 +793,25 @@
                     } else {
                         const float unit_t = 1.0f - a;
                         float depth_t;
+#if AIC_MATERIAL_LOG2 && AIC_POW_BRANCHLESS
+                        depth_t = powf_from_log2_select(__hiloint2double((int)__float_as_uint(rec_mat.y), (int)__float_as_uint(rec_mat.x)), thickness, s_pow);
+                        depth_t = unit_t == 1.0f ? 1.0f : depth_t;
+#else
                         if (unit_t == 0.0f) depth_t = 0.0f;
                         else if (unit_t == 1.0f) depth_t = 1.0f;
                         else if (!(thickness < __uint_as_float(0x7f800000u))) depth_t = 0.0f;
+#if AIC_MATERIAL_LOG2
+                        else depth_t = powf_from_log2(__hiloint2double((int)__float_as_uint(rec_mat.y), (int)__float_as_uint(rec_mat.x)), thickness, s_pow);
+#else
                         else depth_t = powf_table(unit_t, thickness, s_pow);
+#endif
+#endif
                         a = zo_clamped(1.0f - depth_t);
+#if AIC_MATERIAL_RCP
+                        const float ec = (unit_t == 1.0f) ? thickness : div_by_rcp(depth_t - 1.f, unit_t - 1.f, rec_mat.z);
+#else
                         const float ec = (unit_t == 1.0f) ? thickness : (depth_t - 1.f) / (unit_t - 1.f);
+#endif
                         coeff = fmaxf(ec, 0.0f);
                     }
                     const float c = ps_clamped(coeff);
diff --git a/all_is_cubes_amd/csrc/aic_tunables.h b/all_is_cubes_amd/csrc/aic_tunables.h
--- a/all_is_cubes_amd/csrc/aic_tunables.h
+++ b/all_is_cubes_amd/csrc/aic_tunables.h
@@ -34,6 +34,20 @@
 #define AIC_BONUS_MIN 1
 #endif
 
+#ifndef AIC_MATERIAL_LOG2
+#define AIC_MATERIAL_LOG2 1
+#endif
+#ifndef AIC_MATERIAL_RCP
+#define AIC_MATERIAL_RCP 1
+#endif
+
+#ifndef AIC_POW_BRANCHLESS
+#define AIC_POW_BRANCHLESS 1
+#endif
+#ifndef AIC_REC_SELECT
+#define AIC_REC_SELECT 1
+#endif
+
 #ifndef AIC_XWG_THREADS
 #define AIC_XWG_THREADS 256
 #endif
```

New measurement: 6623 (median of 6 runs). Within noise of the previous version (+0.6%).
